# theblackcat102/edgedict

Hardware: NVIDIA H100
Metric: audio-sec/sec E6D2 B=32 T=1000 U=128 V=1024 training step (higher is better)
Workload: dtype bf16

## Files before the change

edgedict_b200/csrc/common.cuh:

```cuda
#pragma once
#include <cuda_runtime.h>
#include <cuda_bf16.h>
#include <stdint.h>
#include <stdio.h>
#include <math.h>

#define EB_OK 0
#define EB_ERR_INVALID 2
#define EB_ERR_CUDA 3

#define EB_API extern "C" __attribute__((visibility("default")))

#define EB_CHECK_LAUNCH()                                                             \
    do {                                                                              \
        cudaError_t e__ = cudaGetLastError();                                         \
        if (e__ != cudaSuccess) {                                                     \
            fprintf(stderr, "[edgedict_b200] %s:%d CUDA error: %s\n", __FILE__,       \
                    __LINE__, cudaGetErrorString(e__));                               \
            return EB_ERR_CUDA;                                                       \
        }                                                                             \
    } while (0)

#define EB_CUDA(call)                                                                 \
    do {                                                                              \
        cudaError_t e__ = (call);                                                     \
        if (e__ != cudaSuccess) {                                                     \
            fprintf(stderr, "[edgedict_b200] %s:%d CUDA error: %s\n", __FILE__,       \
                    __LINE__, cudaGetErrorString(e__));                               \
            return EB_ERR_CUDA;                                                       \
        }                                                                             \
    } while (0)

static inline int eb_num_sms() {
    static int n = 0;
    if (n == 0) {
        int dev = 0;
        cudaGetDevice(&dev);
        cudaDeviceGetAttribute(&n, cudaDevAttrMultiProcessorCount, dev);
        if (n <= 0) n = 132;
    }
    return n;
}

__device__ __forceinline__ float warp_max(float v) {
#pragma unroll
    for (int o = 16; o > 0; o >>= 1) v = fmaxf(v, __shfl_xor_sync(0xffffffffu, v, o));
    return v;
}
__device__ __forceinline__ double warp_max(double v) {
#pragma unroll
    for (int o = 16; o > 0; o >>= 1) v = fmax(v, __shfl_xor_sync(0xffffffffu, v, o));
    return v;
}
template <typename T>
__device__ __forceinline__ T warp_sum(T v) {
#pragma unroll
    for (int o = 16; o > 0; o >>= 1) v += __shfl_xor_sync(0xffffffffu, v, o);
    return v;
}

template <typename T>
__device__ __forceinline__ T block_sum(T v, T* sh ) {
    const int lane = threadIdx.x & 31, w = threadIdx.x >> 5;
    v = warp_sum(v);
    __syncthreads();
    if (lane == 0) sh[w] = v;
    __syncthreads();
    const int nw = (blockDim.x + 31) >> 5;
    T r = (threadIdx.x < nw) ? sh[threadIdx.x] : T(0);
    if (w == 0) {
        r = warp_sum(r);
        if (lane == 0) sh[32] = r;
    }
    __syncthreads();
    return sh[32];
}

__device__ __forceinline__ void spin_wait_ge(const unsigned* ctr, unsigned target) {
    unsigned v;
    long long t0 = 0;
    unsigned spins = 0;
    while (true) {
        asm volatile("ld.acquire.gpu.global.u32 %0, [%1];" : "=r"(v) : "l"(ctr) : "memory");
        if (v >= target) break;
        if ((++spins & 0xFFFF) == 0) {
            const long long now = clock64();
            if (t0 == 0) t0 = now;
            else if (now - t0 > 8000000000LL) {
                printf("[edgedict_b200] grid barrier timeout: block %d saw %u, wants %u\n", blockIdx.x, v, target);
                __trap();
            }
        }
    }
}

__device__ __forceinline__ float fast_ex2(float x) {
    float y;
    asm("ex2.approx.ftz.f32 %0, %1;" : "=f"(y) : "f"(x));
    return y;
}
__device__ __forceinline__ float fast_exp(float x) { return fast_ex2(x * 1.4426950408889634f); }
__device__ __forceinline__ float sigmoidf_(float x) { return 1.0f / (1.0f + expf(-x)); }

__device__ __forceinline__ float4 ld_stream_f4(const float* p) {
    float4 r;
    asm volatile("ld.global.nc.L1::no_allocate.v4.f32 {%0,%1,%2,%3}, [%4];"
                 : "=f"(r.x), "=f"(r.y), "=f"(r.z), "=f"(r.w) : "l"(p));
    return r;
}
__device__ __forceinline__ void st_stream_f4(float* p, float4 v) {
    asm volatile("st.global.L1::no_allocate.v4.f32 [%0], {%1,%2,%3,%4};"
                 :: "l"(p), "f"(v.x), "f"(v.y), "f"(v.z), "f"(v.w) : "memory");
}
```

edgedict_b200/csrc/gemm_tc.cu:

```cuda
#include <cuda.h>
#include <stdlib.h>
#include "common.cuh"
#include "sm90.cuh"
#include "../../include/edgedict_b200.h"

namespace {

constexpr int BM = 128, BK = 64, UMMA_K = 16;
constexpr int A_BYTES = BM * BK * 2;
constexpr int NTHREADS = 2 * 128 + 32;
template <int BN_, bool LOW_ = false> struct Cfg {
    static constexpr int STAGES = LOW_ ? 3 : (BN_ == 256 ? 4 : 6);
    static constexpr int B_BYTES = BN_ * BK * 2;
    static constexpr int STAGE_BYTES = A_BYTES + B_BYTES;
    static constexpr int SMEM_BYTES = 1024 + STAGES * STAGE_BYTES + 256;
};

struct Sched {
    long num_m; int num_n; int ksplit; long out_tiles; bool n_inner;
    unsigned wid, nw;
    __device__ __forceinline__ bool get(long j, long& m_blk, int& n_blk, int& ks) const {
        if (n_inner) {
            const long grp = (long)wid + (j / num_n) * nw;
            if (grp >= num_m) return false;
            m_blk = grp; n_blk = (int)(j % num_n); ks = 0;
            return true;
        }
        const long wi = (long)wid + j * nw;
        if (wi >= out_tiles * ksplit) return false;
        const long tile = wi % out_tiles;
        ks = (int)(wi / out_tiles);
        m_blk = tile / num_n; n_blk = (int)(tile % num_n);
        return true;
    }
};

struct LseArgs {
    const int* labels; const int* xlen; const int* ylen;
    float* denom; float* lpb; float* lpl;
    int maxT, maxU, blank;
    const __nv_bfloat16* aux;
};

__device__ __forceinline__ void st_bf16x2(__nv_bfloat16* p, float a, float b) {
    *reinterpret_cast<__nv_bfloat162*>(p) = __floats2bfloat162_rn(a, b);
}

template <bool A_MN, bool B_MN, int BN_, bool LSE = false, bool LOW_ = false>
__global__ void __launch_bounds__(NTHREADS, LOW_ ? 2 : 1)
gemm_tc_kernel(const __grid_constant__ CUtensorMap tma_a, const __grid_constant__ CUtensorMap tma_b,
               void* __restrict__ Cout, int c_bf16, const float* __restrict__ bias, int accumulate,
               long M, int N, long K, int ksplit, LseArgs lse = LseArgs(), float* __restrict__ part = nullptr) {
    using C_ = Cfg<BN_, LOW_>;
    constexpr int BN = BN_, STAGES = C_::STAGES, STAGE_BYTES = C_::STAGE_BYTES, NACC = BN / 2;
    extern __shared__ uint8_t smem_raw[];
    uint8_t* smem = reinterpret_cast<uint8_t*>((reinterpret_cast<uintptr_t>(smem_raw) + 1023) & ~uintptr_t(1023));
    uint8_t* tiles = smem;
    uint64_t* bars = reinterpret_cast<uint64_t*>(smem + STAGES * STAGE_BYTES);
    const uint32_t full0 = smem_u32(bars), empty0 = smem_u32(bars + STAGES);

    const int warp = threadIdx.x >> 5, lane = threadIdx.x & 31;
    const long num_m = (M + BM - 1) / BM;
    const int num_n = (N + BN - 1) / BN;
    Sched sch;
    sch.num_m = num_m; sch.num_n = num_n; sch.ksplit = ksplit; sch.out_tiles = num_m * num_n;
    sch.wid = blockIdx.x; sch.nw = gridDim.x;
    sch.n_inner = LSE || ((ksplit == 1) && (num_m >= 2L * sch.nw));
    const int nkb_total = (int)((K + BK - 1) / BK);
    const int kb_per = (nkb_total + ksplit - 1) / ksplit;

    if (threadIdx.x == 0) {
        for (int s = 0; s < STAGES; ++s) { mbar_init(full0 + 8 * s, 1); mbar_init(empty0 + 8 * s, 8); }
        asm volatile("fence.mbarrier_init.release.cluster;" ::: "memory");
        asm volatile("prefetch.tensormap [%0];" :: "l"(&tma_a) : "memory");
        asm volatile("prefetch.tensormap [%0];" :: "l"(&tma_b) : "memory");
    }
    __syncthreads();

    if (warp == 8) {
        if (lane == 0) {
            int stage = 0; uint32_t phase = 0;
            long mb; int nb, ksx;
            constexpr uint32_t TX = A_BYTES + C_::B_BYTES;
            for (long jj = 0; sch.get(jj, mb, nb, ksx); ++jj) {
                const int kb0 = ksx * kb_per, kb1 = min(nkb_total, kb0 + kb_per);
                const int m0 = (int)mb * BM, n0 = nb * BN;
                for (int kb = kb0; kb < kb1; ++kb) {
                    mbar_wait(empty0 + 8 * stage, phase ^ 1);
                    const uint32_t sa = smem_u32(tiles + stage * STAGE_BYTES), sb = sa + A_BYTES;
                    const uint32_t fb = full0 + 8 * stage;
                    mbar_expect_tx(fb, TX);
                    if (!A_MN) tma_load_2d(sa, &tma_a, kb * BK, m0, fb);
                    else { tma_load_2d(sa, &tma_a, m0, kb * BK, fb); tma_load_2d(sa + 8192, &tma_a, m0 + 64, kb * BK, fb); }
                    if (!B_MN) tma_load_2d(sb, &tma_b, kb * BK, n0, fb);
                    else {
#pragma unroll
                        for (int bx = 0; bx < BN / 64; ++bx) tma_load_2d(sb + bx * 8192, &tma_b, n0 + bx * 64, kb * BK, fb);
                    }
                    if (++stage == STAGES) { stage = 0; phase ^= 1; }
                }
            }
        }
        return;
    }

    const int wg = warp >> 2;
    const int r_in = 64 * wg + 16 * (warp & 3) + (lane >> 2);
    const int cq = 2 * (lane & 3);
    float* Cf = reinterpret_cast<float*>(Cout);
    __nv_bfloat16* const Ch = reinterpret_cast<__nv_bfloat16*>(Cout);
    const bool vec2 = (N % 2) == 0;
    float acc[NACC];
    int stage = 0; uint32_t phase = 0;
    long mb; int nb, ks;
    float rm[2] = {-INFINITY, -INFINITY}, rs[2] = {0.f, 0.f}, xb[2] = {0.f, 0.f}, xl[2] = {0.f, 0.f};
    int lab[2] = {-1, -1};
    bool cell_ok[2] = {false, false};
    for (long jj = 0; sch.get(jj, mb, nb, ks); ++jj) {
        const int kb0 = ks * kb_per, kb1 = min(nkb_total, kb0 + kb_per);
        const long m0 = mb * BM;
        const int n0 = nb * BN;
#pragma unroll
        for (int i = 0; i < NACC; ++i) acc[i] = 0.f;
        int prev = -1;
        for (int kb = kb0; kb < kb1; ++kb) {
            mbar_wait(full0 + 8 * stage, phase);
            const uint32_t sa = smem_u32(tiles + stage * STAGE_BYTES) + (uint32_t)wg * 8192u, sb = smem_u32(tiles + stage * STAGE_BYTES) + A_BYTES;
            wgmma_fence();
#pragma unroll
            for (int k = 0; k < BK / UMMA_K; ++k) {
                const uint64_t ad = A_MN ? make_desc(sa + k * 2048, 8192, 1024) : make_desc(sa + k * 32, 16, 1024);
                const uint64_t bd = B_MN ? make_desc(sb + k * 2048, 8192, 1024) : make_desc(sb + k * 32, 16, 1024);
                if constexpr (BN == 256) wgmma_m64n256k16<A_MN ? 1 : 0, B_MN ? 1 : 0>(acc, ad, bd, 1);
                else wgmma_m64n128k16<A_MN ? 1 : 0, B_MN ? 1 : 0>(acc, ad, bd, 1);
            }
            wgmma_commit();
            wgmma_wait<1>();
            if (prev >= 0 && lane == 0) mbar_arrive(empty0 + 8 * prev);
            prev = stage;
            if (++stage == STAGES) { stage = 0; phase ^= 1; }
        }
        wgmma_wait<0>();
        wgmma_fence_regs(acc);
        if (prev >= 0 && lane == 0) mbar_arrive(empty0 + 8 * prev);

        if constexpr (LSE) {
            constexpr float LOG2E = 1.4426950408889634f;
            if (nb == 0) {
#pragma unroll
                for (int h = 0; h < 2; ++h) {
                    rm[h] = -INFINITY; rs[h] = 0.f; xb[h] = 0.f; xl[h] = 0.f; lab[h] = -1; cell_ok[h] = false;
                    const long cell = m0 + r_in + 8 * h;
                    if (cell < M) {
                        const int u = (int)(cell % lse.maxU);
                        const long bt = cell / lse.maxU;
                        const int t = (int)(bt % lse.maxT), b = (int)(bt / lse.maxT);
                        const int Tn = lse.xlen[b], Un = lse.ylen[b] + 1;
                        cell_ok[h] = t < Tn && u < Un;
                        if (cell_ok[h] && u < Un - 1) lab[h] = lse.labels[b * (lse.maxU - 1) + u];
                    }
                }
            }
#pragma unroll
            for (int h = 0; h < 2; ++h) {
                float cm = -INFINITY;
#pragma unroll
                for (int i = 0; i < BN / 8; ++i) {
                    const int col = n0 + 8 * i + cq;
                    float v0 = acc[4 * i + 2 * h], v1 = acc[4 * i + 2 * h + 1];
                    v0 = col < N ? v0 + (bias ? __ldg(bias + col) : 0.f) : -INFINITY;
                    v1 = col + 1 < N ? v1 + (bias ? __ldg(bias + col + 1) : 0.f) : -INFINITY;
                    acc[4 * i + 2 * h] = v0; acc[4 * i + 2 * h + 1] = v1;
                    cm = fmaxf(cm, fmaxf(v0, v1));
                    if (col == lse.blank) xb[h] = v0;
                    if (col + 1 == lse.blank) xb[h] = v1;
                    if (col == lab[h]) xl[h] = v0;
                    if (col + 1 == lab[h]) xl[h] = v1;
                }
                const float nm = fmaxf(rm[h], cm);
                if (nm != -INFINITY) {
                    const float nml = nm * LOG2E;
                    float a0 = 0.f, a1 = 0.f;
#pragma unroll
                    for (int i = 0; i < BN / 8; ++i) {
                        a0 += fast_ex2(fmaf(acc[4 * i + 2 * h], LOG2E, -nml));
                        a1 += fast_ex2(fmaf(acc[4 * i + 2 * h + 1], LOG2E, -nml));
                    }
                    rs[h] = rs[h] * fast_ex2((rm[h] - nm) * LOG2E) + (a0 + a1);
                    rm[h] = nm;
                }
                const long row = m0 + r_in + 8 * h;
                if (row < M) {
#pragma unroll
                    for (int i = 0; i < BN / 8; ++i) {
                        const int col = n0 + 8 * i + cq;
                        __nv_bfloat16* cp = Ch + row * N + col;
                        if (vec2 && col + 1 < N) st_bf16x2(cp, acc[4 * i + 2 * h], acc[4 * i + 2 * h + 1]);
                        else {
                            if (col < N) cp[0] = __float2bfloat16(acc[4 * i + 2 * h]);
                            if (col + 1 < N) cp[1] = __float2bfloat16(acc[4 * i + 2 * h + 1]);
                        }
                    }
                }
            }
            if (nb == num_n - 1) {
#pragma unroll
                for (int h = 0; h < 2; ++h) {
#pragma unroll
                    for (int o = 1; o <= 2; o <<= 1) {
                        const float m2 = __shfl_xor_sync(0xffffffffu, rm[h], o), s2 = __shfl_xor_sync(0xffffffffu, rs[h], o);
                        xb[h] += __shfl_xor_sync(0xffffffffu, xb[h], o);
                        xl[h] += __shfl_xor_sync(0xffffffffu, xl[h], o);
                        const float m = fmaxf(rm[h], m2);
                        rs[h] = (rm[h] == -INFINITY ? 0.f : rs[h] * fast_ex2((rm[h] - m) * LOG2E)) +
                                (m2 == -INFINITY ? 0.f : s2 * fast_ex2((m2 - m) * LOG2E));
                        rm[h] = m;
                    }
                    if ((lane & 3) == 0 && cell_ok[h]) {
                        const long cell = m0 + r_in + 8 * h;
                        const float d = -(rm[h] + logf(rs[h]));
                        lse.denom[cell] = d;
                        lse.lpb[cell] = d + xb[h];
                        lse.lpl[cell] = d + xl[h];
                    }
                }
            }
        } else {
            const bool add_bias = bias && ks == 0;
            if (ksplit > 1) Cf = part + (long)ks * M * N;
            const int acc_c = ksplit > 1 ? 0 : accumulate;
#pragma unroll
            for (int h = 0; h < 2; ++h) {
                const long row = m0 + r_in + 8 * h;
                if (row >= M) continue;
                constexpr bool PRE = BN == 128 && !LOW_;
                __nv_bfloat162 hx[PRE ? BN / 8 : 1];
                if constexpr (PRE) {
                    if (c_bf16 && lse.aux) {
#pragma unroll
                        for (int i = 0; i < BN / 8; ++i) {
                            const int col = n0 + 8 * i + cq;
                            const long off = row * N + col;
                            hx[i] = __floats2bfloat162_rn(0.f, 0.f);
                            if (col + 1 < N && vec2) hx[i] = __ldg(reinterpret_cast<const __nv_bfloat162*>(lse.aux + off));
                            else if (col < N) {
                                hx[i].x = lse.aux[off];
                                if (col + 1 < N) hx[i].y = lse.aux[off + 1];
                            }
                        }
                    }
                }
#pragma unroll
                for (int i = 0; i < BN / 8; ++i) {
                    const int col = n0 + 8 * i + cq;
                    if (col >= N) break;
                    const bool two = col + 1 < N, pair = two && vec2;
                    float v0 = acc[4 * i + 2 * h], v1 = acc[4 * i + 2 * h + 1];
                    if (add_bias) { v0 += __ldg(bias + col); if (two) v1 += __ldg(bias + col + 1); }
                    const long off = row * N + col;
                    if (c_bf16) {
                        __nv_bfloat16* cp = Ch + off;
                        if (lse.aux) {
                            float h0, h1 = 0.f;
                            if constexpr (PRE) {
                                const float2 hh = __bfloat1622float2(hx[i]);
                                h0 = hh.x;
                                if (two) h1 = hh.y;
                            } else if (pair) {
                                const float2 hh = __bfloat1622float2(__ldg(reinterpret_cast<const __nv_bfloat162*>(lse.aux + off)));
                                h0 = hh.x; h1 = hh.y;
                            } else {
                                h0 = __bfloat162float(lse.aux[off]);
                                if (two) h1 = __bfloat162float(lse.aux[off + 1]);
                            }
                            v0 *= 1.f - h0 * h0; v1 *= 1.f - h1 * h1;
                        }
                        if (pair) {
                            if (accumulate) {
                                const float2 o = __bfloat1622float2(*reinterpret_cast<const __nv_bfloat162*>(cp));
                                v0 += o.x; v1 += o.y;
                            }
                            st_bf16x2(cp, v0, v1);
                        } else {
                            if (accumulate) { v0 += __bfloat162float(cp[0]); if (two) v1 += __bfloat162float(cp[1]); }
                            cp[0] = __float2bfloat16(v0);
                            if (two) cp[1] = __float2bfloat16(v1);
                        }
                    } else {
                        float* cp = Cf + off;
                        if (pair) {
                            if (acc_c) { const float2 o = *reinterpret_cast<const float2*>(cp); v0 += o.x; v1 += o.y; }
                            *reinterpret_cast<float2*>(cp) = make_float2(v0, v1);
                        } else {
                            if (acc_c) { v0 += cp[0]; if (two) v1 += cp[1]; }
                            cp[0] = v0;
                            if (two) cp[1] = v1;
                        }
                    }
                }
            }
        }
    }
}

__global__ void splitk_reduce_kernel(const float* __restrict__ part, int ksplit, long mn, float* __restrict__ C, int accumulate) {
    for (long i = (long)blockIdx.x * blockDim.x + threadIdx.x; i < mn; i += (long)gridDim.x * blockDim.x) {
        float v = accumulate ? C[i] : 0.f;
        for (int s = 0; s < ksplit; ++s) v += part[(long)s * mn + i];
        C[i] = v;
    }
}

int choose_ksplit(long out_tiles, long nkb, long workers, double r) {
    int ksplit = 1;
    long cap = nkb / 16;
    if (cap > 64) cap = 64;
    double best = -1.0;
    for (long ks = 1; ks <= cap; ++ks) {
        const long items = out_tiles * ks;
        const long waves = (items + workers - 1) / workers;
        const double score = (double)items / (double)(waves * workers) / (1.0 + r * (double)ks / (double)nkb);
        if (score > best) { best = score; ksplit = (int)ks; }
    }
    return ksplit;
}

template <bool A_MN, bool B_MN, int BN_, bool LSE, bool LOW_>
int launch_kernel(const CUtensorMap& ta, const CUtensorMap& tb, void* C, int c_bf16, const float* bias, int accumulate,
                  long M, int N, long K, int ksplit, long work, const LseArgs& ea, cudaStream_t st, float* part = nullptr) {
    using C_ = Cfg<BN_, LOW_>;
    auto kern = gemm_tc_kernel<A_MN, B_MN, BN_, LSE, LOW_>;
    static bool attr_done = false;
    if (!attr_done) {
        EB_CUDA(cudaFuncSetAttribute(kern, cudaFuncAttributeMaxDynamicSharedMemorySize, C_::SMEM_BYTES));
        attr_done = true;
    }
    const int grid = (int)(work < eb_num_sms() ? work : eb_num_sms());
    kern<<<grid, NTHREADS, C_::SMEM_BYTES, st>>>(ta, tb, C, c_bf16, bias, accumulate, M, N, K, ksplit, ea, part);
    EB_CHECK_LAUNCH();
    if (ksplit > 1) {
        const long mn = M * (long)N;
        const long blocks = (mn + 255) / 256, cap = 4L * eb_num_sms();
        splitk_reduce_kernel<<<(int)(blocks < cap ? blocks : cap), 256, 0, st>>>(part, ksplit, mn, (float*)C, accumulate);
        EB_CHECK_LAUNCH();
    }
    return EB_OK;
}

template <bool A_MN, bool B_MN, int BN_>
int launch(const CUtensorMap& ta, const CUtensorMap& tb, void* C, int c_bf16, const float* bias, int accumulate,
           long M, int N, long K, int ksplit, float* part, cudaStream_t st, const void* aux = nullptr) {
    LseArgs ea = LseArgs();
    ea.aux = reinterpret_cast<const __nv_bfloat16*>(aux);
    const long out_tiles = ((M + BM - 1) / BM) * ((N + BN_ - 1) / BN_);
    return launch_kernel<A_MN, B_MN, BN_, false, false>(ta, tb, C, c_bf16, bias, accumulate, M, N, K, ksplit,
                                                        out_tiles * ksplit, ea, st, part);
}

void plan(int a_mn_major, int c_bf16, int accumulate, long M, int N, long K, int flags, bool& wide, int& ksplit) {
    const bool low = (flags & EB_GEMM_CORESIDENT) != 0;
    static int force_bn = -1;
    if (force_bn < 0) { const char* e = getenv("EDGEDICT_GEMM_BN"); force_bn = e ? atoi(e) : 0; }
    const long wide_tiles = ((M + BM - 1) / BM) * (N / 256);
    wide = (N % 256 == 0) && (wide_tiles >= eb_num_sms() || (!c_bf16 && (K + BK - 1) / BK >= 64 && wide_tiles >= 8));
    if (!wide && N % 256 == 128 && N >= 512 && (M + BM - 1) / BM >= 4L * eb_num_sms() && accumulate == 0) wide = true;
    if (force_bn == 128) wide = false;
    if (force_bn == 256 && N % 128 == 0) wide = true;
    if (low) wide = false;
    (void)a_mn_major;
    const int BN = wide ? 256 : 128;
    const long out_tiles = ((M + BM - 1) / BM) * ((N + BN - 1) / BN);
    const long nkb = (K + BK - 1) / BK;
    ksplit = 1;
    if (!low && !c_bf16 && nkb >= 64 && out_tiles < eb_num_sms())
        ksplit = choose_ksplit(out_tiles, nkb, eb_num_sms(), BN == 256 ? 32.0 : 16.0);
}

int launch_low(const CUtensorMap& ta, const CUtensorMap& tb, void* C, int c_bf16, const float* bias, int accumulate,
               long M, int N, long K, cudaStream_t st) {
    const long tiles = ((M + BM - 1) / BM) * ((N + 127) / 128);
    return launch_kernel<false, false, 128, false, true>(ta, tb, C, c_bf16, bias, accumulate, M, N, K, 1, tiles, LseArgs(), st);
}

int launch_lse(const CUtensorMap& ta, const CUtensorMap& tb, void* C, const float* bias, long M, int N, long K,
               const LseArgs& lse, cudaStream_t st) {
    return launch_kernel<false, false, 128, true, false>(ta, tb, C, 1, bias, 0, M, N, K, 1, (M + BM - 1) / BM, lse, st);
}

}

EB_API int eb_joint_logits_lse(const void* hidden16, const void* w2_16, const float* b2, void* logits16,
                               const int* labels, const int* xlen, const int* ylen, float* denom, float* lpb,
                               float* lpl, int B, int maxT, int maxU, int V, int J, int blank, void* stream) {
    if (!hidden16 || !w2_16 || !logits16 || !xlen || !ylen || !denom || !lpb || !lpl || (!labels && maxU > 1) ||
        B <= 0 || maxT <= 0 || maxU <= 0 || V <= 0 || J <= 0 || J % 8 || blank < 0 || blank >= V)
        return EB_ERR_INVALID;
    if ((reinterpret_cast<uintptr_t>(hidden16) & 15) || (reinterpret_cast<uintptr_t>(w2_16) & 15) ||
        (b2 && (reinterpret_cast<uintptr_t>(b2) & 15)))
        return EB_ERR_INVALID;
    const long M = (long)B * maxT * maxU;
    CUtensorMap ta, tb;
    if (!make_map(&ta, hidden16, (uint64_t)J, (uint64_t)M, 128) || !make_map(&tb, w2_16, (uint64_t)J, (uint64_t)V, 128)) {
        fprintf(stderr, "[edgedict_b200] cuTensorMapEncodeTiled failed\n");
        return EB_ERR_CUDA;
    }
    LseArgs lse;
    lse.labels = labels; lse.xlen = xlen; lse.ylen = ylen; lse.denom = denom; lse.lpb = lpb; lse.lpl = lpl;
    lse.maxT = maxT; lse.maxU = maxU; lse.blank = blank; lse.aux = nullptr;
    cudaStream_t st = reinterpret_cast<cudaStream_t>(stream);
    return launch_lse(ta, tb, logits16, b2, M, V, J, lse, st);
}

EB_API int eb_gemm_bf16(const void* A, int a_mn_major, const void* B, int b_mn_major, void* C, int c_bf16,
                        const float* bias, int accumulate, long M, int N, long K, void* stream) {
    return eb_gemm_bf16_ex(A, a_mn_major, B, b_mn_major, C, c_bf16, bias, accumulate, M, N, K, 0, nullptr, 0, stream);
}

static int gemm_dispatch(const void* A, int a_mn_major, const void* B, int b_mn_major, void* C, int c_bf16,
                         const float* bias, int accumulate, long M, int N, long K, int flags, const void* aux,
                         float* partials, long partial_floats, void* stream);

EB_API long eb_gemm_bf16_partials(int a_mn_major, int c_bf16, int accumulate, long M, int N, long K, int flags) {
    if (M <= 0 || N <= 0 || K <= 0) return 0;
    bool wide;
    int ksplit;
    plan(a_mn_major, c_bf16, accumulate, M, N, K, flags, wide, ksplit);
    return ksplit > 1 ? (long)ksplit * M * N : 0;
}

EB_API int eb_gemm_bf16_ex(const void* A, int a_mn_major, const void* B, int b_mn_major, void* C, int c_bf16,
                           const float* bias, int accumulate, long M, int N, long K, int flags, float* partials,
                           long partial_floats, void* stream) {
    return gemm_dispatch(A, a_mn_major, B, b_mn_major, C, c_bf16, bias, accumulate, M, N, K, flags, nullptr, partials,
                         partial_floats, stream);
}

EB_API int eb_gemm_bf16_dtanh(const void* A, int a_mn_major, const void* B, int b_mn_major, void* C16,
                              const void* hid16, long M, int N, long K, void* stream) {
    if (!hid16 || (reinterpret_cast<uintptr_t>(hid16) & 7) || (reinterpret_cast<uintptr_t>(C16) & 7) || N % 4) return EB_ERR_INVALID;
    return gemm_dispatch(A, a_mn_major, B, b_mn_major, C16, 1, nullptr, 0, M, N, K, 0, hid16, nullptr, 0, stream);
}

static int gemm_dispatch(const void* A, int a_mn_major, const void* B, int b_mn_major, void* C, int c_bf16,
                         const float* bias, int accumulate, long M, int N, long K, int flags, const void* aux,
                         float* partials, long partial_floats, void* stream) {
    if (!A || !B || !C || M <= 0 || N <= 0 || K <= 0) return EB_ERR_INVALID;
    const bool low = (flags & EB_GEMM_CORESIDENT) != 0;
    if (low && (a_mn_major || b_mn_major)) return EB_ERR_INVALID;
    if ((reinterpret_cast<uintptr_t>(A) & 15) || (reinterpret_cast<uintptr_t>(B) & 15)) return EB_ERR_INVALID;
    if ((a_mn_major ? M : K) % 8 || (b_mn_major ? (long)N : K) % 8) return EB_ERR_INVALID;
    bool wide;
    int ksplit;
    plan(a_mn_major, c_bf16, accumulate, M, N, K, flags, wide, ksplit);
    if (aux) wide = false;
    if (ksplit > 1) {
        const long fit = (partials && (reinterpret_cast<uintptr_t>(partials) & 7) == 0) ? partial_floats / (M * (long)N) : 0;
        if (fit < ksplit) ksplit = fit > 1 ? (int)fit : 1;
    }
    CUtensorMap ta, tb;
    bool ok = a_mn_major ? make_map(&ta, A, (uint64_t)M, (uint64_t)K, 64) : make_map(&ta, A, (uint64_t)K, (uint64_t)M, 128);
    ok = ok && (b_mn_major ? make_map(&tb, B, (uint64_t)N, (uint64_t)K, 64)
                           : make_map(&tb, B, (uint64_t)K, (uint64_t)N, wide ? 256 : 128));
    if (!ok) {
        fprintf(stderr, "[edgedict_b200] cuTensorMapEncodeTiled failed\n");
        return EB_ERR_CUDA;
    }
    cudaStream_t st = reinterpret_cast<cudaStream_t>(stream);
    if (low) return launch_low(ta, tb, C, c_bf16, bias, accumulate, M, N, K, st);
#define EB_GO(AM, BMN)                                                                                          \
    return wide ? launch<AM, BMN, 256>(ta, tb, C, c_bf16, bias, accumulate, M, N, K, ksplit, partials, st, aux) \
                : launch<AM, BMN, 128>(ta, tb, C, c_bf16, bias, accumulate, M, N, K, ksplit, partials, st, aux)
    if (a_mn_major) {
        if (b_mn_major) { EB_GO(true, true); }
        EB_GO(true, false);
    }
    if (b_mn_major) { EB_GO(false, true); }
    EB_GO(false, false);
#undef EB_GO
}
```

edgedict_b200/csrc/sm90.cuh:

```cuda
#pragma once
#include <cuda.h>
#include "common.cuh"

namespace {

__device__ __forceinline__ uint32_t smem_u32(const void* p) { return (uint32_t)__cvta_generic_to_shared(p); }

__device__ __forceinline__ void mbar_init(uint32_t bar, uint32_t count) {
    asm volatile("mbarrier.init.shared::cta.b64 [%0], %1;" :: "r"(bar), "r"(count) : "memory");
}
__device__ __forceinline__ void mbar_expect_tx(uint32_t bar, uint32_t bytes) {
    asm volatile("mbarrier.arrive.expect_tx.shared::cta.b64 _, [%0], %1;" :: "r"(bar), "r"(bytes) : "memory");
}
__device__ __forceinline__ void mbar_arrive(uint32_t bar) {
    asm volatile("mbarrier.arrive.shared::cta.b64 _, [%0];" :: "r"(bar) : "memory");
}
__device__ __forceinline__ void mbar_wait(uint32_t bar, uint32_t parity) {
    uint32_t ok = 0;
    unsigned long long spins = 0;
    do {
        asm volatile("{\n .reg .pred p;\n mbarrier.try_wait.parity.shared::cta.b64 p, [%1], %2;\n"
                     " selp.u32 %0, 1, 0, p;\n}\n" : "=r"(ok) : "r"(bar), "r"(parity) : "memory");
        if (!ok && ++spins > (1ull << 26)) {
            printf("[edgedict_b200] mbarrier wait timeout (block %d warp %d)\n", blockIdx.x,
                   threadIdx.x >> 5);
            __trap();
        }
    } while (!ok);
}
__device__ __forceinline__ void tma_load_2d(uint32_t dst, const CUtensorMap* map, int c0, int c1, uint32_t bar) {
    asm volatile("cp.async.bulk.tensor.2d.shared::cluster.global.mbarrier::complete_tx::bytes [%0], [%1, {%3, %4}], [%2];"
                 :: "r"(dst), "l"(map), "r"(bar), "r"(c0), "r"(c1) : "memory");
}

__device__ __forceinline__ void wgmma_fence() { asm volatile("wgmma.fence.sync.aligned;" ::: "memory"); }
__device__ __forceinline__ void wgmma_commit() { asm volatile("wgmma.commit_group.sync.aligned;" ::: "memory"); }
template <int N>
__device__ __forceinline__ void wgmma_wait() { asm volatile("wgmma.wait_group.sync.aligned %0;" :: "n"(N) : "memory"); }
template <int R>
__device__ __forceinline__ void wgmma_fence_regs(float (&d)[R]) {
#pragma unroll
    for (int i = 0; i < R; ++i) asm volatile("" : "+f"(d[i]) :: "memory");
}
template <int TA, int TB>
__device__ __forceinline__ void wgmma_m64n32k16(float (&d)[16], uint64_t da, uint64_t db, int scale_d) {
    asm volatile("{\n .reg .pred p;\n setp.ne.b32 p, %18, 0;\n"
                 " wgmma.mma_async.sync.aligned.m64n32k16.f32.bf16.bf16 {"
                 "%0,%1,%2,%3,%4,%5,%6,%7,%8,%9,%10,%11,%12,%13,%14,%15"
                 "}, %16, %17, p, 1, 1, %19, %20;\n}\n"
                 : "+f"(d[0]), "+f"(d[1]), "+f"(d[2]), "+f"(d[3]), "+f"(d[4]), "+f"(d[5]), "+f"(d[6]), "+f"(d[7]),
                   "+f"(d[8]), "+f"(d[9]), "+f"(d[10]), "+f"(d[11]), "+f"(d[12]), "+f"(d[13]), "+f"(d[14]), "+f"(d[15])
                 : "l"(da), "l"(db), "r"(scale_d), "n"(TA), "n"(TB));
}
template <int TA, int TB>
__device__ __forceinline__ void wgmma_m64n128k16(float (&d)[64], uint64_t da, uint64_t db, int scale_d) {
    asm volatile("{\n .reg .pred p;\n setp.ne.b32 p, %66, 0;\n"
                 " wgmma.mma_async.sync.aligned.m64n128k16.f32.bf16.bf16 {"
                 "%0,%1,%2,%3,%4,%5,%6,%7,%8,%9,%10,%11,%12,%13,%14,%15,"
                 "%16,%17,%18,%19,%20,%21,%22,%23,%24,%25,%26,%27,%28,%29,%30,%31,"
                 "%32,%33,%34,%35,%36,%37,%38,%39,%40,%41,%42,%43,%44,%45,%46,%47,"
                 "%48,%49,%50,%51,%52,%53,%54,%55,%56,%57,%58,%59,%60,%61,%62,%63"
                 "}, %64, %65, p, 1, 1, %67, %68;\n}\n"
                 : "+f"(d[0]), "+f"(d[1]), "+f"(d[2]), "+f"(d[3]), "+f"(d[4]), "+f"(d[5]), "+f"(d[6]), "+f"(d[7]),
                   "+f"(d[8]), "+f"(d[9]), "+f"(d[10]), "+f"(d[11]), "+f"(d[12]), "+f"(d[13]), "+f"(d[14]), "+f"(d[15]),
                   "+f"(d[16]), "+f"(d[17]), "+f"(d[18]), "+f"(d[19]), "+f"(d[20]), "+f"(d[21]), "+f"(d[22]), "+f"(d[23]),
                   "+f"(d[24]), "+f"(d[25]), "+f"(d[26]), "+f"(d[27]), "+f"(d[28]), "+f"(d[29]), "+f"(d[30]), "+f"(d[31]),
                   "+f"(d[32]), "+f"(d[33]), "+f"(d[34]), "+f"(d[35]), "+f"(d[36]), "+f"(d[37]), "+f"(d[38]), "+f"(d[39]),
                   "+f"(d[40]), "+f"(d[41]), "+f"(d[42]), "+f"(d[43]), "+f"(d[44]), "+f"(d[45]), "+f"(d[46]), "+f"(d[47]),
                   "+f"(d[48]), "+f"(d[49]), "+f"(d[50]), "+f"(d[51]), "+f"(d[52]), "+f"(d[53]), "+f"(d[54]), "+f"(d[55]),
                   "+f"(d[56]), "+f"(d[57]), "+f"(d[58]), "+f"(d[59]), "+f"(d[60]), "+f"(d[61]), "+f"(d[62]), "+f"(d[63])
                 : "l"(da), "l"(db), "r"(scale_d), "n"(TA), "n"(TB));
}
template <int TA, int TB>
__device__ __forceinline__ void wgmma_m64n256k16(float (&d)[128], uint64_t da, uint64_t db, int scale_d) {
    asm volatile("{\n .reg .pred p;\n setp.ne.b32 p, %130, 0;\n"
                 " wgmma.mma_async.sync.aligned.m64n256k16.f32.bf16.bf16 {"
                 "%0,%1,%2,%3,%4,%5,%6,%7,%8,%9,%10,%11,%12,%13,%14,%15,"
                 "%16,%17,%18,%19,%20,%21,%22,%23,%24,%25,%26,%27,%28,%29,%30,%31,"
                 "%32,%33,%34,%35,%36,%37,%38,%39,%40,%41,%42,%43,%44,%45,%46,%47,"
                 "%48,%49,%50,%51,%52,%53,%54,%55,%56,%57,%58,%59,%60,%61,%62,%63,"
                 "%64,%65,%66,%67,%68,%69,%70,%71,%72,%73,%74,%75,%76,%77,%78,%79,"
                 "%80,%81,%82,%83,%84,%85,%86,%87,%88,%89,%90,%91,%92,%93,%94,%95,"
                 "%96,%97,%98,%99,%100,%101,%102,%103,%104,%105,%106,%107,%108,%109,%110,%111,"
                 "%112,%113,%114,%115,%116,%117,%118,%119,%120,%121,%122,%123,%124,%125,%126,%127"
                 "}, %128, %129, p, 1, 1, %131, %132;\n}\n"
                 : "+f"(d[0]), "+f"(d[1]), "+f"(d[2]), "+f"(d[3]), "+f"(d[4]), "+f"(d[5]), "+f"(d[6]), "+f"(d[7]),
                   "+f"(d[8]), "+f"(d[9]), "+f"(d[10]), "+f"(d[11]), "+f"(d[12]), "+f"(d[13]), "+f"(d[14]), "+f"(d[15]),
                   "+f"(d[16]), "+f"(d[17]), "+f"(d[18]), "+f"(d[19]), "+f"(d[20]), "+f"(d[21]), "+f"(d[22]), "+f"(d[23]),
                   "+f"(d[24]), "+f"(d[25]), "+f"(d[26]), "+f"(d[27]), "+f"(d[28]), "+f"(d[29]), "+f"(d[30]), "+f"(d[31]),
                   "+f"(d[32]), "+f"(d[33]), "+f"(d[34]), "+f"(d[35]), "+f"(d[36]), "+f"(d[37]), "+f"(d[38]), "+f"(d[39]),
                   "+f"(d[40]), "+f"(d[41]), "+f"(d[42]), "+f"(d[43]), "+f"(d[44]), "+f"(d[45]), "+f"(d[46]), "+f"(d[47]),
                   "+f"(d[48]), "+f"(d[49]), "+f"(d[50]), "+f"(d[51]), "+f"(d[52]), "+f"(d[53]), "+f"(d[54]), "+f"(d[55]),
                   "+f"(d[56]), "+f"(d[57]), "+f"(d[58]), "+f"(d[59]), "+f"(d[60]), "+f"(d[61]), "+f"(d[62]), "+f"(d[63]),
                   "+f"(d[64]), "+f"(d[65]), "+f"(d[66]), "+f"(d[67]), "+f"(d[68]), "+f"(d[69]), "+f"(d[70]), "+f"(d[71]),
                   "+f"(d[72]), "+f"(d[73]), "+f"(d[74]), "+f"(d[75]), "+f"(d[76]), "+f"(d[77]), "+f"(d[78]), "+f"(d[79]),
                   "+f"(d[80]), "+f"(d[81]), "+f"(d[82]), "+f"(d[83]), "+f"(d[84]), "+f"(d[85]), "+f"(d[86]), "+f"(d[87]),
                   "+f"(d[88]), "+f"(d[89]), "+f"(d[90]), "+f"(d[91]), "+f"(d[92]), "+f"(d[93]), "+f"(d[94]), "+f"(d[95]),
                   "+f"(d[96]), "+f"(d[97]), "+f"(d[98]), "+f"(d[99]), "+f"(d[100]), "+f"(d[101]), "+f"(d[102]), "+f"(d[103]),
                   "+f"(d[104]), "+f"(d[105]), "+f"(d[106]), "+f"(d[107]), "+f"(d[108]), "+f"(d[109]), "+f"(d[110]), "+f"(d[111]),
                   "+f"(d[112]), "+f"(d[113]), "+f"(d[114]), "+f"(d[115]), "+f"(d[116]), "+f"(d[117]), "+f"(d[118]), "+f"(d[119]),
                   "+f"(d[120]), "+f"(d[121]), "+f"(d[122]), "+f"(d[123]), "+f"(d[124]), "+f"(d[125]), "+f"(d[126]), "+f"(d[127])
                 : "l"(da), "l"(db), "r"(scale_d), "n"(TA), "n"(TB));
}


__device__ __forceinline__ uint64_t make_desc(uint32_t saddr, uint32_t lbo_bytes, uint32_t sbo_bytes) {
    uint64_t d = 0;
    d |= (uint64_t)((saddr & 0x3FFFF) >> 4);
    d |= (uint64_t)((lbo_bytes >> 4) & 0x3FFF) << 16;
    d |= (uint64_t)((sbo_bytes >> 4) & 0x3FFF) << 32;
    d |= (uint64_t)1 << 62;
    return d;
}


__device__ __forceinline__ uint32_t cluster_ctarank() {
    uint32_t r;
    asm volatile("mov.u32 %0, %%cluster_ctarank;" : "=r"(r));
    return r;
}
__device__ __forceinline__ uint32_t map_to_rank(uint32_t saddr, uint32_t rank) {
    uint32_t r;
    asm volatile("mapa.shared::cluster.u32 %0, %1, %2;" : "=r"(r) : "r"(saddr), "r"(rank));
    return r;
}
__device__ __forceinline__ void st_cluster_f4(uint32_t caddr, float a, float b, float c, float d) {
    asm volatile("st.shared::cluster.v4.f32 [%0], {%1,%2,%3,%4};" :: "r"(caddr), "f"(a), "f"(b), "f"(c), "f"(d) : "memory");
}
__device__ __forceinline__ void mbar_arrive_cluster(uint32_t caddr) {
    asm volatile("mbarrier.arrive.release.cluster.shared::cluster.b64 _, [%0];" :: "r"(caddr) : "memory");
}
__device__ __forceinline__ void mbar_wait_cluster(uint32_t bar, uint32_t parity) {
    uint32_t ok = 0;
    unsigned long long spins = 0;
    do {
        asm volatile("{\n .reg .pred p;\n mbarrier.try_wait.parity.acquire.cluster.shared::cta.b64 p, [%1], %2;\n"
                     " selp.u32 %0, 1, 0, p;\n}\n" : "=r"(ok) : "r"(bar), "r"(parity) : "memory");
        if (!ok && ++spins > (1ull << 26)) {
            printf("[edgedict_b200] cluster mbarrier wait timeout (block %d warp %d)\n", blockIdx.x, threadIdx.x >> 5);
            __trap();
        }
    } while (!ok);
}
__device__ __forceinline__ void cluster_sync_all() {
    asm volatile("barrier.cluster.arrive.release.aligned;\nbarrier.cluster.wait.acquire.aligned;" ::: "memory");
}
__device__ __forceinline__ void fence_proxy_async() { asm volatile("fence.proxy.async;" ::: "memory"); }

__device__ __forceinline__ void bulk_s2c(uint32_t dst_cluster, uint32_t src_cta, uint32_t bytes, uint32_t mbar_cluster) {
    asm volatile("cp.async.bulk.shared::cluster.shared::cta.mbarrier::complete_tx::bytes [%0], [%1], %2, [%3];"
                 :: "r"(dst_cluster), "r"(src_cta), "r"(bytes), "r"(mbar_cluster) : "memory");
}
__device__ __forceinline__ void fence_proxy_async_smem() { asm volatile("fence.proxy.async.shared::cta;" ::: "memory"); }

typedef CUresult (*EncodeTiledFn)(CUtensorMap*, CUtensorMapDataType, cuuint32_t, void*, const cuuint64_t*,
                                  const cuuint64_t*, const cuuint32_t*, const cuuint32_t*,
                                  CUtensorMapInterleave, CUtensorMapSwizzle, CUtensorMapL2promotion,
                                  CUtensorMapFloatOOBfill);

inline EncodeTiledFn get_encode() {
    static EncodeTiledFn fn = nullptr;
    if (!fn) {
        void* p = nullptr;
        cudaDriverEntryPointQueryResult q;
        if (cudaGetDriverEntryPoint("cuTensorMapEncodeTiled", &p, cudaEnableDefault, &q) != cudaSuccess ||
            q != cudaDriverEntryPointSuccess)
            return nullptr;
        fn = reinterpret_cast<EncodeTiledFn>(p);
    }
    return fn;
}

inline bool make_map(CUtensorMap* map, const void* ptr, uint64_t inner, uint64_t outer, uint32_t box_outer) {
    EncodeTiledFn enc = get_encode();
    if (!enc) return false;
    cuuint64_t dims[2] = {inner, outer};
    cuuint64_t strides[1] = {inner * 2};
    cuuint32_t box[2] = {64, box_outer};
    cuuint32_t estr[2] = {1, 1};
    CUresult r = enc(map, CU_TENSOR_MAP_DATA_TYPE_BFLOAT16, 2, const_cast<void*>(ptr), dims, strides, box, estr,
                     CU_TENSOR_MAP_INTERLEAVE_NONE, CU_TENSOR_MAP_SWIZZLE_128B, CU_TENSOR_MAP_L2_PROMOTION_L2_256B,
                     CU_TENSOR_MAP_FLOAT_OOB_FILL_NONE);
    return r == CUDA_SUCCESS;
}

}
```

edgedict_b200/functional.py:

```python
import torch

from . import ops

import os

f32, bf16 = torch.float32, torch.bfloat16
FUSE_JOINT_LSE = os.environ.get("EDGEDICT_FUSE_LSE", "1") != "0"


def _c(t):
    return t if t.is_contiguous() else t.contiguous()


class Linear(torch.autograd.Function):

    @staticmethod
    def forward(ctx, x, w, b, precision):
        shp = x.shape
        x2 = _c(x).view(-1, shp[-1])
        x16 = ops.cast_bf16(x2) if precision == "bf16" else None
        y = ops.mm_nt(x2, w, b, precision, x16=x16)
        ctx.save_for_backward(x2 if x16 is None else x16, w)
        ctx.precision, ctx.has_b, ctx.shp = precision, b is not None, shp
        return y.view(*shp[:-1], w.shape[0])

    @staticmethod
    def backward(ctx, dy):
        xs, w = ctx.saved_tensors
        p = ctx.precision
        dy2 = _c(dy).view(-1, dy.shape[-1])
        dy16 = ops.cast_bf16(dy2) if p == "bf16" else None
        dx = dw = db = None
        if ctx.needs_input_grad[0]:
            dx = ops.mm_nn(dy2, w, p, dy16=dy16).view(ctx.shp)
        if ctx.needs_input_grad[1]:
            dw = ops.mm_tn(dy2, xs, p, dy16=dy16, x16=xs if p == "bf16" else None)
        if ctx.has_b and ctx.needs_input_grad[2]:
            db = ops.colsum(dy2)
        return dx, dw, db, None


class LayerNormRes(torch.autograd.Function):

    @staticmethod
    def forward(ctx, x, res, gamma, beta, eps):
        x = _c(x)
        res = _c(res) if res is not None else None
        y, _, mean, rstd = ops.layernorm_fwd(x, res, gamma, beta, eps)
        ctx.save_for_backward(x, res, gamma, mean, rstd)
        return y

    @staticmethod
    def backward(ctx, dy):
        x, res, gamma, mean, rstd = ctx.saved_tensors
        dz, dgamma, dbeta = ops.layernorm_bwd(_c(dy), x, res, gamma, mean, rstd)
        return dz, (dz if res is not None else None), dgamma, dbeta, None


class TimeReduce(torch.autograd.Function):

    @staticmethod
    def forward(ctx, x):
        ctx.T = x.shape[1]
        y, _ = ops.time_reduce_fwd(_c(x))
        return y

    @staticmethod
    def backward(ctx, dy):
        return ops.time_reduce_bwd(_c(dy), ctx.T)


class Embedding(torch.autograd.Function):

    @staticmethod
    def forward(ctx, ids, w, prepend_bos, bos, pad):
        ids = _c(ids)
        if ids.dtype not in (torch.int32, torch.int64):
            ids = ids.long()
        ctx.save_for_backward(ids)
        ctx.meta = (w.shape[0], prepend_bos, bos, pad)
        return ops.embedding_fwd(ids, w, prepend_bos, bos)

    @staticmethod
    def backward(ctx, dout):
        (ids,) = ctx.saved_tensors
        V, prepend_bos, bos, pad = ctx.meta
        return None, ops.embedding_bwd(ids, _c(dout), V, prepend_bos, bos, pad), None, None, None


C4_BPTT_MIN_H = 1024


def _c4_bptt(H):
    return H >= C4_BPTT_MIN_H and ops.lstm_c4_bwd_chunks_supported(H)


class LSTMLayer(torch.autograd.Function):

    @staticmethod
    def forward(ctx, x, h0, c0, w_ih, w_hh, b_ih, b_hh, precision):
        B, T, I = x.shape
        H = w_hh.shape[1]
        x2 = _c(x).view(B * T, I)
        x16 = ops.cast_bf16(x2) if precision == "bf16" else None
        bias = b_ih + b_hh
        xg = ops.mm_nt(x2, w_ih, bias, precision, x16=x16).view(B, T, 4 * H)
        h0c = _c(h0) if h0 is not None else None
        c0c = _c(c0) if c0 is not None else None
        need = any(ctx.needs_input_grad)
        tc = precision == "bf16" and ops.lstm_tc_supported(B, H)
        c4 = precision == "bf16" and ops.lstm_c4_supported(B, H)
        if c4:
            y, y16, hT, cT, gates, cseq = ops.lstm_c4_fwd(xg, ops.cast_bf16(_c(w_hh)), h0c, c0c, need,
                                                          std_saves=None if ops.C4_BWD else True)
        elif tc:
            y, y16, hT, cT, gates, cseq = ops.lstm_tc_fwd(xg, ops.cast_bf16(_c(w_hh)), h0c, c0c, need)
        else:
            y, hT, cT, gates, cseq = ops.lstm_seq_fwd(xg, _c(w_hh), h0c, c0c, need)
            y16 = None
        if need:
            ctx.save_for_backward(x2 if x16 is None else x16, h0c, c0c, w_ih, w_hh, y16 if (tc or c4) else y, gates, cseq)
            ctx.precision, ctx.dims, ctx.tc, ctx.c4, ctx.c4_bwd = precision, (B, T, I, H), tc, c4, c4 and ops.C4_BWD
        return y, hT, cT

    @staticmethod
    def backward(ctx, dy, dhT, dcT):
        xs, h0, c0, w_ih, w_hh, y, gates, cseq = ctx.saved_tensors
        B, T, I, H = ctx.dims
        p = ctx.precision
        dy = _c(dy) if dy is not None else torch.zeros(B, T, H, dtype=f32, device=y.device)
        dhT = _c(dhT) if dhT is not None else None
        dcT = _c(dcT) if dcT is not None else None
        if getattr(ctx, "consumed", False):
            raise RuntimeError("LSTMLayer.backward ran twice on the same graph: the saved gates are overwritten in "
                               "place by the first pass (retain_graph is not supported by this node)")
        ctx.consumed = True
        if ctx.c4_bwd:
            dg16, dh0, dc0 = ops.lstm_c4_bwd(dy, gates, cseq, c0, ops.transpose_to_bf16(_c(w_hh)), dhT, dcT)
            dg2 = dg16.view(B * T, 4 * H)
        elif ctx.c4 and _c4_bptt(H):
            dg16, dh0, dc0 = ops.lstm_c4_bwd_chunks(dy, gates, cseq, ops.transpose_to_bf16(_c(w_hh)), [T], B,
                                                    torch.empty(B, T, 4 * H, dtype=bf16, device=dy.device), c0, dhT, dcT)
            dg2 = dg16.view(B * T, 4 * H)
        elif ctx.tc or ctx.c4:
            dg16, dh0, dc0 = ops.lstm_tc_bwd(dy, gates, cseq, c0, ops.transpose_to_bf16(_c(w_hh)), dhT, dcT)
            dg2 = dg16.view(B * T, 4 * H)
        else:
            dg, dh0, dc0 = ops.lstm_seq_bwd(dy, gates, cseq, c0, _c(w_hh), dhT, dcT)
            dg2 = dg.view(B * T, 4 * H)
            dg16 = ops.cast_bf16(dg2) if p == "bf16" else None
        dg16 = dg16.view(B * T, 4 * H) if dg16 is not None else None
        if ctx.c4:
            hp2 = y.view(B * T, H)
        else:
            hprev = torch.empty_like(y)
            hprev[:, 1:] = y[:, :-1]
            if h0 is not None:
                hprev[:, 0] = h0
            else:
                hprev[:, 0].zero_()
            hp2 = hprev.view(B * T, H)
        dx = ops.mm_nn(dg2, w_ih, p, dy16=dg16).view(B, T, I) if ctx.needs_input_grad[0] else None
        dw_ih = ops.mm_tn(dg2, xs, p, dy16=dg16, x16=xs if p == "bf16" else None)
        dw_hh = ops.mm_tn(dg2, hp2, p, dy16=dg16, x16=hp2 if hp2.dtype == bf16 else None)
        db = ops.colsum(dg2)
        return (dx, dh0 if ctx.needs_input_grad[1] else None, dc0 if ctx.needs_input_grad[2] else None,
                dw_ih, dw_hh, db, db.clone(), None)


class GRULayer(torch.autograd.Function):

    @staticmethod
    def forward(ctx, x, h0, w_ih, w_hh, b_ih, b_hh, precision):
        B, T, I = x.shape
        H = w_hh.shape[1]
        x2 = _c(x).view(B * T, I)
        x16 = ops.cast_bf16(x2) if precision == "bf16" else None
        bias = torch.cat([b_ih[:2 * H] + b_hh[:2 * H], b_ih[2 * H:]])
        xg = ops.mm_nt(x2, w_ih, bias, precision, x16=x16).view(B, T, 3 * H)
        h0c = _c(h0) if h0 is not None else None
        bhn = _c(b_hh[2 * H:])
        need = any(ctx.needs_input_grad)
        tc = precision == "bf16" and ops.gru_tc_supported(B, H)
        if tc:
            y, hT, save = ops.gru_tc_fwd(xg, ops.cast_bf16(_c(w_hh)), bhn, h0c, need)
        else:
            y, hT, save = ops.gru_seq_fwd(xg, _c(w_hh), bhn, h0c, need)
        if need:
            ctx.save_for_backward(x2 if x16 is None else x16, h0c, w_ih, w_hh, y, save)
            ctx.precision, ctx.dims, ctx.tc = precision, (B, T, I, H), tc
        return y, hT

    @staticmethod
    def backward(ctx, dy, dhT):
        xs, h0, w_ih, w_hh, y, save = ctx.saved_tensors
        B, T, I, H = ctx.dims
        p = ctx.precision
        if getattr(ctx, "consumed", False):
            raise RuntimeError("GRULayer.backward ran twice on the same graph (retain_graph is not supported by this "
                               "node)")
        ctx.consumed = True
        dy = _c(dy) if dy is not None else torch.zeros(B, T, H, dtype=f32, device=y.device)
        dhT = _c(dhT) if dhT is not None else None
        if ctx.tc:
            dgi, dgh, dh0 = ops.gru_tc_bwd(dy, save, y, h0, ops.transpose_to_bf16(_c(w_hh)), dhT)
        else:
            dgi, dgh, dh0 = ops.gru_seq_bwd(dy, save, y, h0, _c(w_hh), dhT)
        dgi2, dgh2 = dgi.view(B * T, 3 * H), dgh.view(B * T, 3 * H)
        dgi16 = (dgi2 if ctx.tc else ops.cast_bf16(dgi2)) if p == "bf16" else None
        dgh16 = (dgh2 if ctx.tc else ops.cast_bf16(dgh2)) if p == "bf16" else None
        hprev = torch.empty_like(y)
        hprev[:, 1:] = y[:, :-1]
        if h0 is not None:
            hprev[:, 0] = h0
        else:
            hprev[:, 0].zero_()
        hp2 = hprev.view(B * T, H)
        dx = ops.mm_nn(dgi2, w_ih, p, dy16=dgi16).view(B, T, I) if ctx.needs_input_grad[0] else None
        dw_ih = ops.mm_tn(dgi2, xs, p, dy16=dgi16, x16=xs if p == "bf16" else None)
        dw_hh = ops.mm_tn(dgh2, hp2, p, dy16=dgh16)
        return (dx, dh0 if ctx.needs_input_grad[1] else None, dw_ih, dw_hh, ops.colsum(dgi2), ops.colsum(dgh2), None)


WAVEFRONT_CHUNKS = int(os.environ.get("EDGEDICT_WAVEFRONT_CHUNKS", "6"))
_wave_streams = {}


def _side_streams(device):
    st = _wave_streams.get(device)
    if st is None:
        st = _wave_streams[device] = (torch.cuda.Stream(device), torch.cuda.Stream(device))
    return st


_aux_streams = {}


def _wave_aux_streams(device):
    st = _aux_streams.get(device)
    if st is None:
        st = _aux_streams[device] = tuple(torch.cuda.Stream(device) for _ in range(4))
    return st


def wavefront_plan(T, reductions, max_chunks=None):
    max_chunks = WAVEFRONT_CHUNKS if max_chunks is None else max_chunks
    if max_chunks < 2:
        return None
    gran = 1 << sum(1 for r in reductions if r)
    step = -(-T // (max_chunks * gran)) * gran
    if step < 16 * gran:
        step = 16 * gran
    lens = [min(step, T - t0) for t0 in range(0, T, step)]
    if len(lens) < 2:
        return None
    plan = [lens]
    for r in reductions:
        lens = [(n + 1) // 2 for n in lens] if r else lens
        plan.append(lens)
    return plan


class _Chunks:

    def __init__(self, B, lens):
        self.B, self.lens = B, lens
        self.off = [0]
        for n in lens:
            self.off.append(self.off[-1] + n)
        self.rows = B * self.off[-1]

    def new(self, D, dtype, device):
        return torch.empty(self.rows, D, dtype=dtype, device=device) if D else torch.empty(self.rows, dtype=dtype, device=device)

    def blk(self, buf, c):
        a, b = self.B * self.off[c], self.B * self.off[c + 1]
        v = buf[a:b]
        return v.view(self.B, self.lens[c], buf.shape[1]) if buf.dim() == 2 else v

    def scatter(self, x):
        out = self.new(x.shape[2], x.dtype, x.device)
        for c in range(len(self.lens)):
            self.blk(out, c).copy_(x[:, self.off[c]:self.off[c + 1]])
        return out

    def gather(self, buf):
        out = torch.empty(self.B, self.off[-1], buf.shape[1], dtype=buf.dtype, device=buf.device)
        for c in range(len(self.lens)):
            out[:, self.off[c]:self.off[c + 1]].copy_(self.blk(buf, c))
        return out


BPTT_ONE_LAUNCH = __import__("os").environ.get("EDGEDICT_BPTT_ONE_LAUNCH", "1") != "0"


class LSTMStack(torch.autograd.Function):

    collect = None

    @staticmethod
    def forward(ctx, x, cfg, *params):
        reductions, eps, plan = cfg
        L = len(reductions)
        B, T, I0 = x.shape
        dev = x.device
        H = params[1].shape[1]
        C = len(plan[0])
        need = any(ctx.needs_input_grad)
        c4 = ops.lstm_c4_supported(B, H)
        c4b = c4 and ops.C4_BWD
        ck = [_Chunks(B, lens) for lens in plan]
        P = [params[6 * l:6 * l + 6] for l in range(L)]
        wih16 = [ops.cast_bf16(_c(p[0])) for p in P]
        whh16 = [ops.cast_bf16(_c(p[1])) for p in P]
        bias = [p[2] + p[3] for p in P]
        x16 = [ck[0].scatter(ops.cast_bf16(_c(x)))] + [None] * L
        xs = [None] * (L + 1)
        y, y16, gates, cseq, mean, rstd = ([None] * L for _ in range(6))
        z = [None] * L
        for l in range(L):
            k, kn = ck[l], ck[l + 1]
            y[l] = k.new(H, f32, dev)
            y16[l] = k.new(H, bf16, dev) if (need or not c4) else None
            gates[l] = k.new(4 * H, f32, dev) if (need and not c4b) else None
            cseq[l] = k.new(H, f32, dev) if (need and not c4b) else None
            mean[l], rstd[l] = k.new(0, f32, dev), k.new(0, f32, dev)
            xs[l + 1] = kn.new(H, f32, dev)
            z[l] = k.new(H, f32, dev) if reductions[l] else xs[l + 1]
            x16[l + 1] = kn.new(H, bf16, dev) if l + 1 < L else None
        hT = torch.empty(L, C, B, H, dtype=f32, device=dev)
        cT = torch.empty(L, C, B, H, dtype=f32, device=dev)
        xgbuf = [[torch.empty(B * max(plan[l]), 4 * H, dtype=f32, device=dev) for _ in range(2)] for l in range(L)]
        c4saves = [[None] * C for _ in range(L)]

        main = torch.cuda.current_stream(dev)
        rec = _side_streams(dev)
        aux = _wave_aux_streams(dev)
        gem, nrm = aux[:2], aux[2:]
        ev = lambda: torch.cuda.Event()
        prep_done = [[ev() for _ in range(C)] for _ in range(L)]
        rec_done = [[ev() for _ in range(C)] for _ in range(L)]
        done = [[ev() for _ in range(C)] for _ in range(L)]
        for s_ in (*rec, *aux):
            s_.wait_stream(main)
        for d in range(L + C - 1):
            for l in range(max(0, d - C + 1), min(L, d + 1)):
                c = d - l
                k, kn = ck[l], ck[l + 1]
                Tc = k.lens[c]
                xg = xgbuf[l][c % 2][:B * Tc]
                with torch.cuda.stream(gem[l % 2]):
                    if l > 0:
                        gem[l % 2].wait_event(done[l - 1][c])
                    if c >= 2:
                        gem[l % 2].wait_event(rec_done[l][c - 2])
                    xin = k.blk(x16[l], c)
                    ops.gemm_bf16(xin.view(B * Tc, xin.shape[2]), 0, wih16[l], 0, B * Tc, 4 * H, xin.shape[2],
                                  bias=bias[l], out=xg, flags=ops.GEMM_CORESIDENT)
                    prep_done[l][c].record(gem[l % 2])
                with torch.cuda.stream(rec[l % 2]):
                    rec[l % 2].wait_event(prep_done[l][c])
                    if c4:
                        r = ops.lstm_c4_fwd(xg.view(B, Tc, 4 * H), whh16[l], hT[l, c - 1] if c else None,
                                            cT[l, c - 1] if c else None, need,
                                            out=(k.blk(y[l], c), k.blk(y16[l], c) if need else None, hT[l, c], cT[l, c]),
                                            std_saves=None if (c4b or not need) else (k.blk(gates[l], c), k.blk(cseq[l], c)))
                        if need and c4b:
                            c4saves[l][c] = (r[4], r[5])
                            r[4].record_stream(main)
                            r[5].record_stream(main)
                    else:
                        ops.lstm_tc_fwd(xg.view(B, Tc, 4 * H), whh16[l], hT[l, c - 1] if c else None,
                                        cT[l, c - 1] if c else None, need,
                                        out=(k.blk(y[l], c), k.blk(y16[l], c), hT[l, c], cT[l, c],
                                             k.blk(gates[l], c) if need else None, k.blk(cseq[l], c) if need else None))
                    rec_done[l][c].record(rec[l % 2])
                with torch.cuda.stream(nrm[l % 2]):
                    nrm[l % 2].wait_event(rec_done[l][c])
                    res = k.blk(xs[l], c) if l else None
                    nx16 = kn.blk(x16[l + 1], c) if x16[l + 1] is not None else None
                    if reductions[l]:
                        ops.layernorm_fwd(k.blk(y[l], c), res, P[l][4], P[l][5], eps[l],
                                          out=(k.blk(z[l], c), None, k.blk(mean[l], c), k.blk(rstd[l], c)))
                        ops.time_reduce_fwd(k.blk(z[l], c), out=(kn.blk(xs[l + 1], c), nx16))
                    else:
                        ops.layernorm_fwd(k.blk(y[l], c), res, P[l][4], P[l][5], eps[l],
                                          out=(kn.blk(xs[l + 1], c), nx16, k.blk(mean[l], c), k.blk(rstd[l], c)))
                    done[l][c].record(nrm[l % 2])
        for s_ in (*rec, *aux):
            main.wait_stream(s_)
        out = ck[L].gather(xs[L])
        if LSTMStack.collect is not None:
            LSTMStack.collect.extend(ck[l + 1].gather(xs[l + 1]) for l in range(L))
        hT_last, cT_last = hT[:, C - 1].contiguous(), cT[:, C - 1].contiguous()
        if need:
            if c4b:
                gates = [torch.empty(0, device=dev)] * L
                cseq = [torch.empty(0, device=dev)] * L
            flat_saves = [t for row in c4saves for pair in row for t in pair] if c4b else []
            ctx.save_for_backward(*params, hT, cT, *x16[:L], *xs[1:L], *y, *y16, *gates, *cseq, *mean, *rstd, *flat_saves)
            ctx.cfg, ctx.dims, ctx.c4, ctx.c4b = cfg, (B, T, I0, H, L, C), c4, c4b
        ctx.mark_non_differentiable(hT_last, cT_last)
        return out, hT_last, cT_last

    @staticmethod
    def backward(ctx, dout, _dh, _dc):
        reductions, eps, plan = ctx.cfg
        B, T, I0, H, L, C = ctx.dims
        sv = list(ctx.saved_tensors)
        params, sv = sv[:6 * L], sv[6 * L:]
        hT, cT = sv[0], sv[1]
        sv = sv[2:]
        x16, sv = sv[:L], sv[L:]
        xs, sv = [None] + sv[:L - 1], sv[L - 1:]
        y, y16, gates, cseq, mean, rstd = (sv[i * L:(i + 1) * L] for i in range(6))
        c4, c4b = ctx.c4, ctx.c4b
        flat_saves = sv[6 * L:]
        if getattr(ctx, "consumed", False):
            raise RuntimeError("LSTMStack.backward ran twice on the same graph (retain_graph is not supported)")
        ctx.consumed = True
        P = [params[6 * l:6 * l + 6] for l in range(L)]
        ck = [_Chunks(B, lens) for lens in plan]
        dev = dout.device
        main = torch.cuda.current_stream(dev)
        side = _side_streams(dev)[0]
        side.wait_stream(main)
        g = ck[L].scatter(_c(dout))
        grads = [None] * (6 * L)
        for l in range(L - 1, -1, -1):
            k, kn = ck[l], ck[l + 1]
            if reductions[l]:
                gz = k.new(H, f32, dev)
                for c in range(C):
                    ops.time_reduce_bwd(kn.blk(g, c), k.lens[c], out=k.blk(gz, c))
                g = gz
            dz, dgamma, dbeta = ops.layernorm_bwd(g, y[l], xs[l], P[l][4], mean[l], rstd[l])
            whhT16 = ops.transpose_to_bf16(_c(P[l][1]))
            dg16 = k.new(4 * H, bf16, dev)
            dh = dc = None
            if c4b:
                hprev = y16[l]
                for c in range(C - 1, -1, -1):
                    gs, cs = flat_saves[2 * (l * C + c)], flat_saves[2 * (l * C + c) + 1]
                    _, dh, dc = ops.lstm_c4_bwd(k.blk(dz, c), gs, cs, cT[l, c - 1] if c else None, whhT16, dh, dc,
                                                out=k.blk(dg16, c))
            else:
                hprev = y16[l] if c4 else k.new(H, bf16, dev)
                one_launch = c4 and BPTT_ONE_LAUNCH and C <= 8
                if one_launch and _c4_bptt(H):
                    ops.lstm_c4_bwd_chunks(dz, gates[l], cseq[l], whhT16, k.lens, B, dg16)
                elif one_launch:
                    ops.lstm_tc_bwd_chunks(dz, gates[l], cseq[l], whhT16, k.lens, B, dg16)
                for c in (() if one_launch else range(C - 1, -1, -1)):
                    _, dh, dc = ops.lstm_tc_bwd(k.blk(dz, c), k.blk(gates[l], c), k.blk(cseq[l], c),
                                                cT[l, c - 1] if c else None, whhT16, dh, dc, out=k.blk(dg16, c))
                    if c4:
                        continue
                    hp, yc = k.blk(hprev, c), k.blk(y16[l], c)
                    hp[:, 1:] = yc[:, :-1]
                    if c:
                        hp[:, 0] = k.blk(y16[l], c - 1)[:, -1]
                    else:
                        hp[:, 0].zero_()
            wih16 = ops.cast_bf16(_c(P[l][0]))
            M, I_l = dg16.shape[0], P[l][0].shape[1]
            if l > 0:
                g = ops.gemm_bf16(dg16, 0, wih16, 1, M, I_l, 4 * H, out=dz, accumulate=True, tag="gemm_bf16_nn")
            elif ctx.needs_input_grad[0]:
                g = ops.gemm_bf16(dg16, 0, wih16, 1, M, I_l, 4 * H, tag="gemm_bf16_nn")
            else:
                g = None
            ready = torch.cuda.Event()
            ready.record(main)
            with torch.cuda.stream(side):
                side.wait_event(ready)
                grads[6 * l + 0] = ops.mm_tn(dg16, x16[l], "bf16", dy16=dg16, x16=x16[l])
                grads[6 * l + 1] = ops.mm_tn(dg16, hprev, "bf16", dy16=dg16, x16=hprev)
                db = ops.colsum(dg16)
                grads[6 * l + 2], grads[6 * l + 3] = db, db.clone()
                for t_ in (dg16, hprev):
                    t_.record_stream(side)
                for t_ in grads[6 * l:6 * l + 4]:
                    t_.record_stream(main)
            grads[6 * l + 4], grads[6 * l + 5] = dgamma, dbeta
        main.wait_stream(side)
        dxin = ck[0].gather(g) if g is not None else None
        return (dxin, None, *grads)


def _joint_pre(h_enc, h_dec, w1, b1, precision):
    B, T, E = h_enc.shape
    U, Dd = h_dec.shape[1], h_dec.shape[2]
    J = w1.shape[0]
    he2, hd2 = _c(h_enc).view(B * T, E), _c(h_dec).view(B * U, Dd)
    ep = ops.mm_nt(he2, w1[:, :E], b1, precision).view(B, T, J)
    dp = ops.mm_nt(hd2, w1[:, E:], None, precision).view(B, U, J)
    return he2, hd2, ep, dp


JOINT_WGRAD_SIDE = __import__("os").environ.get("EDGEDICT_JOINT_WGRAD_SIDE", "1") != "0"


def _joint_bwd(ctx_p, dlog2, hid, he2, hd2, w1, w2, dims, db2=None):
    B, T, U, E, Dd, J, V = dims
    p = ctx_p
    dl16 = dlog2 if dlog2.dtype == bf16 else (ops.cast_bf16(dlog2) if p == "bf16" else None)
    hid2 = hid.view(B * T * U, J)

    def out_layer_grads(db2):
        if db2 is None:
            db2 = ops.colsum(dlog2)
        if p == "bf16" and V % 256 == 0:
            dw2 = ops.mm_tn(hid2, dl16, p, dy16=hid2, x16=dl16).t().contiguous()
        else:
            dw2 = ops.mm_tn(dlog2, hid2, p, dy16=dl16, x16=hid2 if p == "bf16" else None)
        return dw2, db2

    side = None
    if JOINT_WGRAD_SIDE and p == "bf16" and dlog2.is_cuda:
        main = torch.cuda.current_stream(dlog2.device)
        side = _side_streams(dlog2.device)[1]
        side.wait_stream(main)
        with torch.cuda.stream(side):
            dw2, db2 = out_layer_grads(db2)
        for t_ in (dlog2, dl16, hid2):
            if t_ is not None:
                t_.record_stream(side)
    else:
        dw2, db2 = out_layer_grads(db2)
    if p == "bf16" and J % 8 == 0 and hid.dtype == bf16:
        dpre = ops.gemm_bf16_dtanh(dl16, ops.cast_bf16(w2.contiguous()), True, hid2, B * T * U, J, V)
        dep, ddp = ops.joint_dpre_reduce(dpre.view(B, T, U, J))
    else:
        dhid = ops.mm_nn(dlog2, w2, p, dy16=dl16, out_bf16=(p == "bf16"))
        dep, ddp = ops.joint_hidden_bwd(dhid.view(B, T, U, J), hid)
    dep2, ddp2 = dep.view(B * T, J), ddp.view(B * U, J)
    w1e, w1d = w1[:, :E], w1[:, E:]
    dhe = ops.mm_nn(dep2, w1e, p).view(B, T, E)
    dhd = ops.mm_nn(ddp2, w1d, p).view(B, U, Dd)
    dw1 = torch.empty_like(w1)
    dw1[:, :E] = ops.mm_tn(dep2, he2, p)
    dw1[:, E:] = ops.mm_tn(ddp2, hd2, p)
    db1 = ops.colsum(dep2)
    if side is not None:
        main.wait_stream(side)
        dw2.record_stream(main)
        db2.record_stream(main)
    return dhe, dhd, dw1, db1, dw2, db2


class JointLogits(torch.autograd.Function):

    @staticmethod
    def forward(ctx, h_enc, h_dec, w1, b1, w2, b2, precision):
        B, T, E = h_enc.shape
        U, Dd = h_dec.shape[1], h_dec.shape[2]
        J, V = w1.shape[0], w2.shape[0]
        he2, hd2, ep, dp = _joint_pre(h_enc, h_dec, w1, b1, precision)
        hid = ops.joint_hidden_fwd(ep, dp, precision == "bf16")
        logits = ops.mm_nt(hid.view(B * T * U, J), w2, b2, precision, x16=hid.view(B * T * U, J) if precision == "bf16" else None)
        ctx.save_for_backward(hid, he2, hd2, w1, w2)
        ctx.precision, ctx.dims = precision, (B, T, U, E, Dd, J, V)
        return logits.view(B, T, U, V)

    @staticmethod
    def backward(ctx, dlogits):
        hid, he2, hd2, w1, w2 = ctx.saved_tensors
        B, T, U, E, Dd, J, V = ctx.dims
        dl2 = _c(dlogits).view(B * T * U, V)
        dhe, dhd, dw1, db1, dw2, db2 = _joint_bwd(ctx.precision, dl2, hid, he2, hd2, w1, w2, ctx.dims)
        return dhe, dhd, dw1, db1, dw2, db2, None


class RNNTLossFn(torch.autograd.Function):

    @staticmethod
    def forward(ctx, acts, labels, act_lens, label_lens, blank, reduction):
        acts = _c(acts)
        costs, ws = ops.rnnt_loss_fwd(acts, labels, act_lens, label_lens, blank, need_beta=True)
        B = acts.shape[0]
        ctx.save_for_backward(acts, labels, act_lens, label_lens, ws)
        ctx.blank, ctx.reduction, ctx.B = blank, reduction, B
        if reduction in ("sum", "mean"):
            costs = costs.sum().unsqueeze(-1)
            if reduction == "mean":
                costs = costs / B
        return costs

    @staticmethod
    def backward(ctx, go):
        acts, labels, act_lens, label_lens, ws = ctx.saved_tensors
        scale = 1.0 / ctx.B if ctx.reduction == "mean" else 1.0
        g = _c(go.to(acts.dtype)).view(-1)
        grads = ops.rnnt_loss_bwd(acts, labels, act_lens, label_lens, ctx.blank, ws, g, scale)
        return grads, None, None, None, None, None


class JointLoss(torch.autograd.Function):

    @staticmethod
    def forward(ctx, h_enc, h_dec, w1, b1, w2, b2, labels, act_lens, label_lens, blank, precision):
        B, T, E = h_enc.shape
        U, Dd = h_dec.shape[1], h_dec.shape[2]
        J, V = w1.shape[0], w2.shape[0]
        he2, hd2, ep, dp = _joint_pre(h_enc, h_dec, w1, b1, precision)
        hid = ops.joint_hidden_fwd(ep, dp, precision == "bf16")
        hid2 = hid.view(B * T * U, J)
        fused = precision == "bf16" and FUSE_JOINT_LSE and J % 8 == 0 and U <= 1024
        if fused:
            b2a = b2 if (b2.is_contiguous() and b2.data_ptr() % 16 == 0) else b2.clone()
            logits, ws = ops.joint_logits_lse(hid2, ops.cast_bf16(w2.contiguous()), b2a, labels, act_lens,
                                              label_lens, B, T, U, blank)
            costs = ops.rnnt_lattice(act_lens, label_lens, B, T, U, ws)
        else:
            logits = ops.mm_nt(hid2, w2, b2, precision, x16=hid2 if precision == "bf16" else None).view(B, T, U, V)
            costs, ws = ops.rnnt_loss_fwd(logits, labels, act_lens, label_lens, blank, need_beta=True)
        ctx.save_for_backward(hid, he2, hd2, w1, w2, logits, labels, act_lens, label_lens, ws)
        ctx.precision, ctx.dims, ctx.blank = precision, (B, T, U, E, Dd, J, V), blank
        ctx.mark_non_differentiable(costs)
        loss = costs.sum().unsqueeze(-1) / B
        ctx.costs = costs
        return loss, costs

    @staticmethod
    def backward(ctx, go, _gc):
        hid, he2, hd2, w1, w2, logits, labels, act_lens, label_lens, ws = ctx.saved_tensors
        if getattr(ctx, "consumed", False):
            raise RuntimeError("JointLoss.backward ran twice on the same graph: the gradient is written in place over "
                               "the saved logits (retain_graph is not supported by this node)")
        ctx.consumed = True
        B, T, U, E, Dd, J, V = ctx.dims
        p = ctx.precision
        g = _c(go.to(f32)).view(-1)
        if logits.dtype == bf16:
            dl = ops.rnnt_loss_bwd_bf16(logits, labels, act_lens, label_lens, ctx.blank, ws, g, 1.0 / B)
        elif p == "bf16":
            dl = ops.rnnt_loss_bwd(logits, labels, act_lens, label_lens, ctx.blank, ws, g, 1.0 / B, out_bf16=True)
        else:
            dl = ops.rnnt_loss_bwd(logits, labels, act_lens, label_lens, ctx.blank, ws, g, 1.0 / B, out=logits)
        dhe, dhd, dw1, db1, dw2, db2 = _joint_bwd(p, dl.view(B * T * U, V), hid, he2, hd2, w1, w2, ctx.dims)
        return dhe, dhd, dw1, db1, dw2, db2, None, None, None, None, None
```

edgedict_b200/ops.py:

```python
import torch

from ._lib import lib
from ._lib import check as _check


def _s():
    return torch.cuda.current_stream().cuda_stream


def _p(t):
    if t is None:
        return None
    if not t.is_cuda:
        raise RuntimeError("edgedict_b200 ops need CUDA tensors (got a %s tensor); there is no CPU path" % t.device)
    return t.data_ptr()


def _need(t, dtype=None, name="tensor"):
    if not t.is_cuda:
        raise RuntimeError("edgedict_b200 ops need CUDA tensors (%s is on %s); there is no CPU path" % (name, t.device))
    if dtype is not None and t.dtype != dtype:
        raise TypeError("%s must be %s, got %s" % (name, dtype, t.dtype))
    if not t.is_contiguous():
        raise ValueError("%s must be contiguous" % name)
    return t


f32, bf16 = torch.float32, torch.bfloat16


class _Prof:

    def __init__(self):
        self.enabled = False
        self.events = []
        self.launches = 0

    def reset(self):
        self.events, self.launches = [], 0

    def summary(self, base=None):
        out, spans = {}, {}
        for name, a, b, nbytes, flops in self.events:
            d = out.setdefault(name, dict(ms=0.0, ms_sum=0.0, calls=0, bytes=0.0, flops=0.0))
            d["ms_sum"] += a.elapsed_time(b)
            d["calls"] += 1
            d["bytes"] += nbytes
            d["flops"] += flops
            if base is not None:
                spans.setdefault(name, []).append((base.elapsed_time(a), base.elapsed_time(b)))
        for name, d in out.items():
            if base is None:
                d["ms"] = d["ms_sum"]
                continue
            tot, cur_s, cur_e = 0.0, None, None
            for s0, e0 in sorted(spans[name]):
                if cur_e is None or s0 > cur_e:
                    if cur_e is not None:
                        tot += cur_e - cur_s
                    cur_s, cur_e = s0, e0
                else:
                    cur_e = max(cur_e, e0)
            if cur_e is not None:
                tot += cur_e - cur_s
            d["ms"] = tot
        return out


PROF = _Prof()


def check(rc, what):
    PROF.launches += 1
    _check(rc, what)


class _timed:
    def __init__(self, name, kernels=1, nbytes=0.0, flops=0.0):
        self.name, self.k, self.nbytes, self.flops = name, kernels, nbytes, flops

    def __enter__(self):
        if PROF.enabled:
            self.a = torch.cuda.Event(enable_timing=True)
            self.a.record()
        return self

    def __exit__(self, *exc):
        PROF.launches += self.k - 1
        if PROF.enabled:
            b = torch.cuda.Event(enable_timing=True)
            b.record()
            PROF.events.append((self.name, self.a, b, self.nbytes, self.flops))
        return False


def cast_bf16(x, out=None):
    _need(x, f32, "x")
    y = out if out is not None else torch.empty(x.shape, dtype=bf16, device=x.device)
    n = x.numel()
    if n:
        check(lib().eb_cast_bf16(_p(x), _p(y), n, _s()), "eb_cast_bf16")
    return y


def gemm_f32(A, sam, sak, B, sbk, sbn, M, N, K, bias=None, out=None, beta=0.0, alpha=1.0):
    if out is None:
        out = torch.empty(M, N, dtype=f32, device=A.device)
    with _timed("gemm_f32", 1, 0.0, 2.0 * M * N * K):
        check(lib().eb_gemm_f32(_p(A), sam, sak, _p(B), sbk, sbn, _p(out), N, _p(bias), M, N, K, alpha, beta, _s()),
              "eb_gemm_f32")
    return out


GEMM_CORESIDENT = 1


def gemm_bf16(A, a_mn, B, b_mn, M, N, K, bias=None, out=None, out_bf16=False, accumulate=False, tag=None, flags=0):
    if out is None:
        out = torch.empty(M, N, dtype=bf16 if out_bf16 else f32, device=A.device)
    name = tag or ("gemm_bf16_%s%s" % ("t" if a_mn else "n", "n" if b_mn else "t"))
    with _timed(name, 1, 2.0 * (M * K + N * K) + out.element_size() * M * N, 2.0 * M * N * K):
        c16 = int(out.dtype == bf16)
        nws = int(lib().eb_gemm_bf16_partials(int(a_mn), c16, int(accumulate), M, N, K, int(flags)))
        ws = torch.empty(nws, dtype=f32, device=A.device) if nws else None
        check(lib().eb_gemm_bf16_ex(_p(A), int(a_mn), _p(B), int(b_mn), _p(out), c16, _p(bias), int(accumulate), M, N, K,
                                    int(flags), _p(ws), nws, _s()), "eb_gemm_bf16")
    return out


def mm_nt(x, w, bias=None, precision="fp32", x16=None, w16=None, out_bf16=False):
    M, K = x.shape
    N = w.shape[0]
    if precision == "bf16":
        x16 = x16 if x16 is not None else (x if x.dtype == bf16 else cast_bf16(x))
        w16 = w16 if w16 is not None else cast_bf16(w.contiguous())
        return gemm_bf16(x16, 0, w16, 0, M, N, K, bias=bias, out_bf16=out_bf16)
    _need(x, f32, "x")
    return gemm_f32(x, K, 1, w, w.stride(1), w.stride(0), M, N, K, bias=bias)


def mm_nn(dy, w, precision="fp32", dy16=None, w16=None, out_bf16=False):
    M, N = dy.shape
    K = w.shape[1]
    if precision == "bf16":
        dy16 = dy16 if dy16 is not None else (dy if dy.dtype == bf16 else cast_bf16(dy))
        w16 = w16 if w16 is not None else cast_bf16(w.contiguous())
        return gemm_bf16(dy16, 0, w16, 1, M, K, N, out_bf16=out_bf16)
    _need(dy, f32, "dy")
    return gemm_f32(dy, N, 1, w, w.stride(0), w.stride(1), M, K, N)


def mm_tn(dy, x, precision="fp32", dy16=None, x16=None, out=None, accumulate=False):
    M, N = dy.shape
    K = x.shape[1]
    if precision == "bf16":
        dy16 = dy16 if dy16 is not None else (dy if dy.dtype == bf16 else cast_bf16(dy))
        x16 = x16 if x16 is not None else (x if x.dtype == bf16 else cast_bf16(x))
        return gemm_bf16(dy16, 1, x16, 1, N, K, M, out=out, accumulate=accumulate)
    _need(dy, f32, "dy")
    _need(x, f32, "x")
    return gemm_f32(dy, 1, N, x, K, 1, N, K, M, out=out, beta=1.0 if accumulate else 0.0)


def colsum(x, out=None):
    rows, N = x.shape
    if out is None:
        out = torch.zeros(N, dtype=f32, device=x.device)
    check(lib().eb_colsum(_p(x), int(x.dtype == bf16), _p(out), rows, N, _s()), "eb_colsum")
    return out


def layernorm_fwd(x, res, gamma, beta, eps=1e-5, want_bf16=False, out=None):
    H = x.shape[-1]
    rows = x.numel() // H
    if out is not None:
        y, y16, mean, rstd = out
    else:
        y = torch.empty_like(x)
        y16 = torch.empty(x.shape, dtype=bf16, device=x.device) if want_bf16 else None
        mean = torch.empty(rows, dtype=f32, device=x.device)
        rstd = torch.empty(rows, dtype=f32, device=x.device)
    check(lib().eb_layernorm_fwd(_p(x), _p(res), _p(gamma), _p(beta), _p(y), _p(y16), _p(mean), _p(rstd),
                                 rows, H, eps, _s()), "eb_layernorm_fwd")
    return y, y16, mean, rstd


def layernorm_bwd(dy, x, res, gamma, mean, rstd):
    H = x.shape[-1]
    rows = x.numel() // H
    dz = torch.empty_like(x)
    dgamma = torch.zeros(H, dtype=f32, device=x.device)
    dbeta = torch.zeros(H, dtype=f32, device=x.device)
    check(lib().eb_layernorm_bwd(_p(dy), _p(x), _p(res), _p(gamma), _p(mean), _p(rstd), _p(dz), _p(dgamma),
                                 _p(dbeta), rows, H, _s()), "eb_layernorm_bwd")
    return dz, dgamma, dbeta


def time_reduce_fwd(x, want_bf16=False, out=None):
    B, T, H = x.shape
    if out is not None:
        y, y16 = out
    else:
        y = torch.empty(B, (T + 1) // 2, H, dtype=f32, device=x.device)
        y16 = torch.empty(y.shape, dtype=bf16, device=x.device) if want_bf16 else None
    check(lib().eb_time_reduce_fwd(_p(x), _p(y), _p(y16), B, T, H, _s()), "eb_time_reduce_fwd")
    return y, y16


def time_reduce_bwd(dy, T, out=None):
    B, _, H = dy.shape
    dx = out if out is not None else torch.empty(B, T, H, dtype=f32, device=dy.device)
    check(lib().eb_time_reduce_bwd(_p(dy), _p(dx), B, T, H, _s()), "eb_time_reduce_bwd")
    return dx


def embedding_fwd(ids, W, prepend_bos, bos):
    B, U = ids.shape
    E = W.shape[1]
    out = torch.empty(B, U + (1 if prepend_bos else 0), E, dtype=f32, device=W.device)
    if out.numel():
        check(lib().eb_embedding_fwd(_p(ids), int(ids.dtype == torch.int64), _p(W), _p(out), None, B, U, E,
                                     int(prepend_bos), bos, _s()), "eb_embedding_fwd")
    return out


def embedding_bwd(ids, dout, V, prepend_bos, bos, pad):
    B, U = ids.shape
    E = dout.shape[-1]
    dW = torch.zeros(V, E, dtype=f32, device=dout.device)
    if dout.numel():
        check(lib().eb_embedding_bwd(_p(ids), int(ids.dtype == torch.int64), _p(dout), _p(dW), B, U, E,
                                     int(prepend_bos), bos, pad, _s()), "eb_embedding_bwd")
    return dW


_scratch = {}


def _lstm_scratch(B, H, device):
    key = (B, H, device, _s())
    t = _scratch.get(key)
    if t is None:
        n = lib().eb_lstm_scratch_bytes(B, H)
        if n == 0:
            raise ValueError("LSTM hidden size %d not supported by the persistent kernel" % H)
        t = torch.zeros(n, dtype=torch.uint8, device=device)
        _scratch[key] = t
    return t


def lstm_seq_fwd(xg, whh, h0, c0, save):
    B, T, H4 = xg.shape
    H = H4 // 4
    dev = xg.device
    y = torch.empty(B, T, H, dtype=f32, device=dev)
    hT = torch.empty(B, H, dtype=f32, device=dev)
    cT = torch.empty(B, H, dtype=f32, device=dev)
    gates = torch.empty(B, T, H4, dtype=f32, device=dev) if save else None
    cseq = torch.empty(B, T, H, dtype=f32, device=dev) if save else None
    with _timed("lstm_seq_fwd", 1, 0.0, 2.0 * B * T * 4 * H * H):
        check(lib().eb_lstm_seq_fwd(_p(xg), _p(whh), _p(h0), _p(c0), _p(y), _p(hT), _p(cT), _p(gates), _p(cseq),
                                    _p(_lstm_scratch(B, H, dev)), B, T, H, _s()), "eb_lstm_seq_fwd")
    return y, hT, cT, gates, cseq


def lstm_seq_bwd(dy, gates, cseq, c0, whh, dhT, dcT):
    B, T, H = dy.shape
    dev = dy.device
    dh0 = torch.empty(B, H, dtype=f32, device=dev)
    dc0 = torch.empty(B, H, dtype=f32, device=dev)
    with _timed("lstm_seq_bwd", 1, 0.0, 2.0 * B * T * 4 * H * H):
        check(lib().eb_lstm_seq_bwd(_p(dy), _p(gates), _p(cseq), _p(c0), _p(whh), _p(dhT), _p(dcT), _p(gates),
                                    _p(dh0), _p(dc0), _p(_lstm_scratch(B, H, dev)), B, T, H, _s()), "eb_lstm_seq_bwd")
    return gates, dh0, dc0


def _gru_scratch(B, H, device):
    key = ("gru", B, H, device, _s())
    t = _scratch.get(key)
    if t is None:
        n = lib().eb_gru_scratch_bytes(B, H)
        if n == 0:
            raise ValueError("GRU hidden size %d not supported by the persistent kernel" % H)
        t = torch.zeros(n, dtype=torch.uint8, device=device)
        _scratch[key] = t
    return t


def gru_seq_fwd(xg, whh, bhn, h0, save):
    B, T, H3 = xg.shape
    H = H3 // 3
    dev = xg.device
    y = torch.empty(B, T, H, dtype=f32, device=dev)
    hT = torch.empty(B, H, dtype=f32, device=dev)
    sv = torch.empty(B, T, 4 * H, dtype=f32, device=dev) if save else None
    with _timed("gru_seq_fwd", 1, 0.0, 2.0 * B * T * 3 * H * H):
        check(lib().eb_gru_seq_fwd(_p(xg), _p(whh), _p(bhn), _p(h0), _p(y), _p(hT), _p(sv),
                                   _p(_gru_scratch(B, H, dev)), B, T, H, _s()), "eb_gru_seq_fwd")
    return y, hT, sv


def gru_seq_bwd(dy, save, y, h0, whh, dhT):
    B, T, H = dy.shape
    dev = dy.device
    dgi = torch.empty(B, T, 3 * H, dtype=f32, device=dev)
    dgh = torch.empty(B, T, 3 * H, dtype=f32, device=dev)
    dh0 = torch.empty(B, H, dtype=f32, device=dev)
    with _timed("gru_seq_bwd", 1, 0.0, 2.0 * B * T * 3 * H * H):
        check(lib().eb_gru_seq_bwd(_p(dy), _p(save), _p(y), _p(h0), _p(whh), _p(dhT), _p(dgi), _p(dgh), _p(dh0),
                                   _p(_gru_scratch(B, H, dev)), B, T, H, _s()), "eb_gru_seq_bwd")
    return dgi, dgh, dh0


def gru_tc_supported(B, H):
    return bool(lib().eb_gru_tc_supported(B, H))


def _gru_tc_scratch(B, H, device):
    key = ("gru_tc", H, device, _s())
    t = _scratch.get(key)
    if t is None:
        t = torch.zeros(lib().eb_gru_tc_scratch_bytes(B, H), dtype=torch.uint8, device=device)
        _scratch[key] = t
    return t


def gru_tc_fwd(xg, whh16, bhn, h0, save):
    B, T, H3 = xg.shape
    H = H3 // 3
    dev = xg.device
    y = torch.empty(B, T, H, dtype=f32, device=dev)
    hT = torch.empty(B, H, dtype=f32, device=dev)
    sv = torch.empty(B, T, 4 * H, dtype=f32, device=dev) if save else None
    with _timed("gru_tc_fwd", 1, 0.0, 2.0 * B * T * 3 * H * H):
        check(lib().eb_gru_tc_fwd(_p(xg), _p(whh16), _p(bhn), _p(h0), _p(y), _p(hT), _p(sv),
                                  _p(_gru_tc_scratch(B, H, dev)), B, T, H, _s()), "eb_gru_tc_fwd")
    return y, hT, sv


def gru_tc_bwd(dy, save, y, h0, whhT16, dhT):
    B, T, H = dy.shape
    dev = dy.device
    dgi = torch.empty(B, T, 3 * H, dtype=bf16, device=dev)
    dgh = torch.empty(B, T, 3 * H, dtype=bf16, device=dev)
    dh0 = torch.empty(B, H, dtype=f32, device=dev)
    with _timed("gru_tc_bwd", 1, 0.0, 2.0 * B * T * 3 * H * H):
        check(lib().eb_gru_tc_bwd(_p(dy), _p(save), _p(y), _p(h0), _p(whhT16), _p(dhT), _p(dgi), _p(dgh), _p(dh0),
                                  _p(_gru_tc_scratch(B, H, dev)), B, T, H, _s()), "eb_gru_tc_bwd")
    return dgi, dgh, dh0


def lstm_tc_supported(B, H):
    return bool(lib().eb_lstm_tc_supported(B, H))


def _lstm_tc_scratch(B, H, device):
    key = ("tc", H, device, _s())
    t = _scratch.get(key)
    if t is None:
        t = torch.zeros(lib().eb_lstm_tc_scratch_bytes(B, H), dtype=torch.uint8, device=device)
        _scratch[key] = t
    return t


def lstm_tc_fwd(xg, whh16, h0, c0, save, out=None):
    B, T, H4 = xg.shape
    H = H4 // 4
    dev = xg.device
    if out is not None:
        y, y16, hT, cT, gates, cseq = out
    else:
        y = torch.empty(B, T, H, dtype=f32, device=dev)
        y16 = torch.empty(B, T, H, dtype=bf16, device=dev)
        hT = torch.empty(B, H, dtype=f32, device=dev)
        cT = torch.empty(B, H, dtype=f32, device=dev)
        gates = torch.empty(B, T, H4, dtype=f32, device=dev) if save else None
        cseq = torch.empty(B, T, H, dtype=f32, device=dev) if save else None
    with _timed("lstm_tc_fwd", 1, 0.0, 2.0 * B * T * 4 * H * H):
        check(lib().eb_lstm_tc_fwd(_p(xg), _p(whh16), _p(h0), _p(c0), _p(y), _p(y16), _p(hT), _p(cT), _p(gates),
                                   _p(cseq), _p(_lstm_tc_scratch(B, H, dev)), B, T, H, _s()), "eb_lstm_tc_fwd")
    return y, y16, hT, cT, gates, cseq


def lstm_tc_bwd(dy, gates, cseq, c0, whhT16, dhT, dcT, out=None):
    B, T, H = dy.shape
    dev = dy.device
    dg16 = out if out is not None else torch.empty(B, T, 4 * H, dtype=bf16, device=dev)
    dh0 = torch.empty(B, H, dtype=f32, device=dev)
    dc0 = torch.empty(B, H, dtype=f32, device=dev)
    with _timed("lstm_tc_bwd", 1, 0.0, 2.0 * B * T * 4 * H * H):
        check(lib().eb_lstm_tc_bwd(_p(dy), _p(gates), _p(cseq), _p(c0), _p(whhT16), _p(dhT), _p(dcT), _p(dg16),
                                   _p(dh0), _p(dc0), _p(_lstm_tc_scratch(B, H, dev)), B, T, H, _s()), "eb_lstm_tc_bwd")
    return dg16, dh0, dc0


def lstm_tc_bwd_chunks(dy, gates, cseq, whhT16, lens, B, out):
    import ctypes
    H = dy.shape[1]
    dev = dy.device
    dh0 = torch.empty(B, H, dtype=f32, device=dev)
    dc0 = torch.empty(B, H, dtype=f32, device=dev)
    arr = (ctypes.c_int * len(lens))(*[int(n) for n in lens])
    with _timed("lstm_tc_bwd", 1, 0.0, 2.0 * B * sum(lens) * 4 * H * H):
        check(lib().eb_lstm_tc_bwd_chunks(_p(dy), _p(gates), _p(cseq), None, _p(whhT16), None, None, _p(out), _p(dh0),
                                          _p(dc0), _p(_lstm_tc_scratch(B, H, dev)), B, arr, len(lens), H, _s()),
              "eb_lstm_tc_bwd_chunks")
    return out, dh0, dc0


_c4_ok = {}


def lstm_c4_supported(B, H):
    v = _c4_ok.get(H)
    if v is None:
        v = _c4_ok[H] = bool(lib().eb_lstm_c4_supported(B, H))
    return v


def _lstm_c4_scratch(B, H, device):
    key = ("c4", H, device, _s())
    t = _scratch.get(key)
    if t is None:
        t = torch.zeros(lib().eb_lstm_c4_scratch_bytes(B, H), dtype=torch.uint8, device=device)
        _scratch[key] = t
    return t


def lstm_c4_save_buffers(B, T, H, device):
    return (torch.empty(lib().eb_lstm_c4_gsave_bytes(B, T, H), dtype=torch.uint8, device=device),
            torch.empty(lib().eb_lstm_c4_csave_bytes(B, T, H), dtype=torch.uint8, device=device))


C4_BWD = __import__("os").environ.get("EDGEDICT_LSTM_C4_BWD", "0") != "0"


def lstm_c4_fwd(xg, whh16, h0, c0, save, out=None, std_saves=None):
    B, T, H4 = xg.shape
    H = H4 // 4
    dev = xg.device
    if out is not None:
        y, hprev16, hT, cT = out
    else:
        y = torch.empty(B, T, H, dtype=f32, device=dev)
        hprev16 = torch.empty(B, T, H, dtype=bf16, device=dev) if save else None
        hT = torch.empty(B, H, dtype=f32, device=dev)
        cT = torch.empty(B, H, dtype=f32, device=dev)
    gsave = csave = gstd = cstd = None
    if save and std_saves is not None and std_saves is not False:
        gstd, cstd = std_saves if isinstance(std_saves, tuple) else (torch.empty(B, T, H4, dtype=f32, device=dev),
                                                                     torch.empty(B, T, H, dtype=f32, device=dev))
    elif save:
        gsave, csave = lstm_c4_save_buffers(B, T, H, dev)
    with _timed("lstm_tc_fwd", 1, 0.0, 2.0 * B * T * 4 * H * H):
        check(lib().eb_lstm_c4_fwd(_p(xg), _p(whh16), _p(h0), _p(c0), _p(y), _p(hprev16), _p(hT), _p(cT), _p(gsave),
                                   _p(csave), _p(gstd), _p(cstd), _p(_lstm_c4_scratch(B, H, dev)), B, T, H, _s()),
              "eb_lstm_c4_fwd")
    if gstd is not None:
        return y, hprev16, hT, cT, gstd, cstd
    return y, hprev16, hT, cT, gsave, csave


_c4_chunks_ok = {}


def lstm_c4_bwd_chunks_supported(H):
    v = _c4_chunks_ok.get(H)
    if v is None:
        v = _c4_chunks_ok[H] = lib().eb_lstm_c4_bwd_chunks_cluster(H) == 16
    return v


def lstm_c4_bwd_chunks(dy, gates, cseq, whhT16, lens, B, out, c0=None, dhT=None, dcT=None):
    import ctypes
    H = dy.shape[-1]
    dev = dy.device
    dh0 = torch.empty(B, H, dtype=f32, device=dev)
    dc0 = torch.empty(B, H, dtype=f32, device=dev)
    arr = (ctypes.c_int * len(lens))(*[int(n) for n in lens])
    with _timed("lstm_tc_bwd", 1, 0.0, 2.0 * B * sum(lens) * 4 * H * H):
        check(lib().eb_lstm_c4_bwd_chunks(_p(dy), _p(gates), _p(cseq), _p(c0), _p(whhT16), _p(dhT), _p(dcT), _p(out),
                                          _p(dh0), _p(dc0), _p(_lstm_c4_scratch(B, H, dev)), B, arr, len(lens), H, _s()),
              "eb_lstm_c4_bwd_chunks")
    return out, dh0, dc0


def lstm_c4_bwd(dy, gsave, csave, c0, whhT16, dhT, dcT, out=None):
    B, T, H = dy.shape
    dev = dy.device
    dg16 = out if out is not None else torch.empty(B, T, 4 * H, dtype=bf16, device=dev)
    dh0 = torch.empty(B, H, dtype=f32, device=dev)
    dc0 = torch.empty(B, H, dtype=f32, device=dev)
    with _timed("lstm_tc_bwd", 1, 0.0, 2.0 * B * T * 4 * H * H):
        check(lib().eb_lstm_c4_bwd(_p(dy), _p(gsave), _p(csave), _p(c0), _p(whhT16), _p(dhT), _p(dcT), _p(dg16),
                                   _p(dh0), _p(dc0), _p(_lstm_c4_scratch(B, H, dev)), B, T, H, _s()), "eb_lstm_c4_bwd")
    return dg16, dh0, dc0


def transpose_to_bf16(x):
    rows, cols = x.shape
    y = torch.empty(cols, rows, dtype=bf16, device=x.device)
    check(lib().eb_transpose_to_bf16(_p(x), int(x.dtype == bf16), _p(y), rows, cols, _s()), "eb_transpose_to_bf16")
    return y


def joint_hidden_fwd(ep, dp, want_bf16):
    B, T, J = ep.shape
    U = dp.shape[1]
    hid = torch.empty(B, T, U, J, dtype=bf16 if want_bf16 else f32, device=ep.device)
    check(lib().eb_joint_hidden_fwd(_p(ep), _p(dp), _p(hid), int(want_bf16), B, T, U, J, _s()), "eb_joint_hidden_fwd")
    return hid


def joint_hidden_bwd(dhid, hid):
    B, T, U, J = hid.shape
    dep = torch.empty(B, T, J, dtype=f32, device=hid.device)
    ddp = torch.empty(B, U, J, dtype=f32, device=hid.device)
    check(lib().eb_joint_hidden_bwd(_p(dhid), _p(hid), int(hid.dtype == bf16), _p(dep), _p(ddp), B, T, U, J, _s()),
          "eb_joint_hidden_bwd")
    return dep, ddp


def gemm_bf16_dtanh(A16, B16, b_mn, hid16, M, N, K):
    out = torch.empty(M, N, dtype=bf16, device=A16.device)
    with _timed("gemm_bf16_n%s" % ("n" if b_mn else "t"), 1, 2.0 * (M * K + N * K) + 4.0 * M * N, 2.0 * M * N * K):
        check(lib().eb_gemm_bf16_dtanh(_p(A16), 0, _p(B16), int(b_mn), _p(out), _p(hid16), M, N, K, _s()),
              "eb_gemm_bf16_dtanh")
    return out


def joint_dpre_reduce(dpre16):
    B, T, U, J = dpre16.shape
    dep = torch.empty(B, T, J, dtype=f32, device=dpre16.device)
    ddp = torch.empty(B, U, J, dtype=f32, device=dpre16.device)
    check(lib().eb_joint_dpre_reduce(_p(dpre16), _p(dep), _p(ddp), B, T, U, J, _s()), "eb_joint_dpre_reduce")
    PROF.launches += 1
    return dep, ddp


def rnnt_workspace(B, T, U, dtype, device):
    n = lib().eb_rnnt_workspace_bytes(B, T, U, 8 if dtype == torch.float64 else 4)
    return torch.empty(n, dtype=torch.uint8, device=device)


def rnnt_loss_fwd(logits, labels, xlen, ylen, blank, need_beta=True):
    B, T, U, V = logits.shape
    ds = 8 if logits.dtype == torch.float64 else 4
    ws = rnnt_workspace(B, T, U, logits.dtype, logits.device)
    costs = torch.empty(B, dtype=logits.dtype, device=logits.device)
    with _timed("rnnt_loss_fwd", 3, float(ds) * B * T * U * V, 0.0):
        check(lib().eb_rnnt_loss_fwd(_p(logits), _p(labels), _p(xlen), _p(ylen), B, T, U, V, blank, ds, _p(ws),
                                     _p(costs), int(need_beta), _s()), "eb_rnnt_loss_fwd")
    return costs, ws


def rnnt_loss_bwd(logits, labels, xlen, ylen, blank, ws, gscale, host_scale, out=None, out_bf16=False):
    B, T, U, V = logits.shape
    ds = 8 if logits.dtype == torch.float64 else 4
    if out is None:
        out = torch.empty(logits.shape, dtype=bf16 if out_bf16 else logits.dtype, device=logits.device)
    per_batch = int(gscale is not None and gscale.numel() > 1)
    with _timed("rnnt_loss_bwd", 1, float(ds + out.element_size()) * B * T * U * V, 0.0):
        check(lib().eb_rnnt_loss_bwd(_p(logits), _p(out), int(out.dtype == bf16), _p(labels), _p(xlen), _p(ylen), B, T,
                                     U, V, blank, ds, _p(ws), _p(gscale), per_batch, float(host_scale), _s()),
              "eb_rnnt_loss_bwd")
    return out


def joint_logits_lse(hid16, w2_16, b2, labels, xlen, ylen, B, T, U, blank):
    V, J = w2_16.shape
    logits16 = torch.empty(B, T, U, V, dtype=bf16, device=hid16.device)
    ws = rnnt_workspace(B, T, U, f32, hid16.device)
    n = B * T * U
    wsf = ws.view(f32)
    N = float(n) * V
    with _timed("joint_logits_lse", 1, 2.0 * n * J + 2.0 * N, 2.0 * N * J):
        check(lib().eb_joint_logits_lse(_p(hid16), _p(w2_16), _p(b2), _p(logits16), _p(labels), _p(xlen), _p(ylen),
                                        _p(wsf[0:n]), _p(wsf[n:2 * n]), _p(wsf[2 * n:3 * n]), B, T, U, V, J, blank,
                                        _s()), "eb_joint_logits_lse")
    return logits16, ws


def rnnt_lattice(xlen, ylen, B, T, U, ws, need_beta=True):
    costs = torch.empty(B, dtype=f32, device=ws.device)
    with _timed("rnnt_loss_fwd", 2, 0.0, 0.0):
        check(lib().eb_rnnt_loss_lattice(_p(xlen), _p(ylen), B, T, U, _p(ws), _p(costs), int(need_beta), _s()),
              "eb_rnnt_loss_lattice")
    return costs


def rnnt_loss_bwd_bf16(logits16, labels, xlen, ylen, blank, ws, gscale, host_scale):
    B, T, U, V = logits16.shape
    per_batch = int(gscale is not None and gscale.numel() > 1)
    with _timed("rnnt_loss_bwd", 1, 4.0 * B * T * U * V, 0.0):
        check(lib().eb_rnnt_loss_bwd_bf16(_p(logits16), _p(logits16), _p(labels), _p(xlen), _p(ylen), B, T, U, V, blank,
                                          _p(ws), _p(gscale), per_batch, float(host_scale), _s()), "eb_rnnt_loss_bwd_bf16")
    return logits16


def adam_step(p, g, m, v, lr, beta1, beta2, eps, weight_decay, step, grad_scale=1.0):
    check(lib().eb_adam_step(_p(p), _p(g), _p(m), _p(v), p.numel(), lr, beta1, beta2, eps, weight_decay, step,
                             grad_scale, _s()), "eb_adam_step")


def adam_step_ex(p, g, m, v, lr, beta1, beta2, eps, weight_decay, step, grad_scale=1.0, sumsq=None, max_norm=0.0,
                 adamw=False):
    check(lib().eb_adam_step_ex(_p(p), _p(g), _p(m), _p(v), p.numel(), lr, beta1, beta2, eps, weight_decay, step,
                                grad_scale, _p(sumsq), float(max_norm or 0.0), int(adamw), _s()), "eb_adam_step_ex")


def sumsq(x, out):
    check(lib().eb_sumsq(_p(x), x.numel(), _p(out), _s()), "eb_sumsq")


def logmel_frontend(x, basis, fbT, n_fft, hop, n_mels, n_stack, preemph, take_log=True, pad_to_divisible=True):
    _need(x, f32, "x")
    B, L = x.shape
    nb = n_fft // 2 + 1
    pad = n_fft // 2
    R = -(-(L + 2 * pad) // hop)
    Lp = R * hop
    F = 1 + L // hop
    seq_len = -(-L // hop)
    dev = x.device
    xp = torch.zeros(B * Lp + n_fft, dtype=f32, device=dev)
    check(lib().eb_fe_preemph_pad(_p(x), _p(xp), B, L, Lp, pad, float(preemph or 0.0), int(preemph is not None), _s()),
          "eb_fe_preemph_pad")
    rows = B * R
    spec = gemm_f32(xp, hop, 1, basis, 2 * nb, 1, rows, 2 * nb, n_fft)
    power = torch.empty(rows, nb, dtype=f32, device=dev)
    check(lib().eb_fe_power(_p(spec), _p(power), rows, nb, _s()), "eb_fe_power")
    mel = gemm_f32(power, nb, 1, fbT, n_mels, 1, rows, n_mels, nb)
    Fs = F if pad_to_divisible else F - F % n_stack
    T = -(-Fs // n_stack)
    out = torch.empty(B, T, n_mels * n_stack, dtype=f32, device=dev)
    check(lib().eb_fe_log_stack(_p(mel), _p(out), B, R, Fs, seq_len, n_mels, n_stack, T, int(take_log), _s()),
          "eb_fe_log_stack")
    return out


def fe_mask(x, spans, axis, fill=0.0):
    _need(x, f32, "x")
    B, D1, D2 = x.shape
    check(lib().eb_fe_mask(_p(x), _p(spans), B, D1, D2, spans.shape[1], axis, float(fill), _s()), "eb_fe_mask")
    return x
```

Before: 11160.

## Add ping-pong warpgroup GEMM kernel for joint LSE and dtanh epilogues

Introduces a dedicated ping-pong kernel with one producer warp and two consumer warpgroups that alternate row blocks. While one warpgroup runs its epilogue, the other runs its MMAs. The joint logits+LSE GEMM and the dhidden*dtanh GEMM now use this kernel instead of the generic persistent kernel with fused epilogues, aiming to hide the heavy exp/reduction and tanh-derivative epilogue work behind tensor-core work. It also strips debug printf from the timeout traps, which may reduce register or code pressure, and adds profiling tags. The risk is extra complexity from named barriers and register reallocation, plus possible occupancy or correctness issues in the new schedule.

Result: faster. 11510, median of 6 (+3.1%).

```diff
diff --git a/edgedict_b200/csrc/common.cuh b/edgedict_b200/csrc/common.cuh
--- a/edgedict_b200/csrc/common.cuh
+++ b/edgedict_b200/csrc/common.cuh
@@ -86,10 +86,7 @@
         if ((++spins & 0xFFFF) == 0) {
             const long long now = clock64();
             if (t0 == 0) t0 = now;
-            else if (now - t0 > 8000000000LL) {
-                printf("[edgedict_b200] grid barrier timeout: block %d saw %u, wants %u\n", blockIdx.x, v, target);
-                __trap();
-            }
+            else if (now - t0 > 8000000000LL) __trap();
         }
     }
 }
diff --git a/edgedict_b200/csrc/gemm_tc.cu b/edgedict_b200/csrc/gemm_tc.cu
--- a/edgedict_b200/csrc/gemm_tc.cu
+++ b/edgedict_b200/csrc/gemm_tc.cu
@@ -46,7 +46,99 @@
     *reinterpret_cast<__nv_bfloat162*>(p) = __floats2bfloat162_rn(a, b);
 }
 
-template <bool A_MN, bool B_MN, int BN_, bool LSE = false, bool LOW_ = false>
+struct LseRows {
+    float rm[2] = {-INFINITY, -INFINITY}, rs[2] = {0.f, 0.f}, xb[2] = {0.f, 0.f}, xl[2] = {0.f, 0.f};
+    int lab[2] = {-1, -1};
+    bool cell_ok[2] = {false, false};
+};
+
+template <int BN>
+__device__ __forceinline__ void lse_epilogue(float (&acc)[BN / 2], LseRows& s, long m0, int r_in, int n0, int nb,
+                                             int num_n, long M, int N, const float* __restrict__ bias,
+                                             __nv_bfloat16* const Ch, const LseArgs& lse, int cq, bool vec2) {
+    constexpr float LOG2E = 1.4426950408889634f;
+    if (nb == 0) {
+#pragma unroll
+        for (int h = 0; h < 2; ++h) {
+            s.rm[h] = -INFINITY; s.rs[h] = 0.f; s.xb[h] = 0.f; s.xl[h] = 0.f; s.lab[h] = -1; s.cell_ok[h] = false;
+            const long cell = m0 + r_in + 8 * h;
+            if (cell < M) {
+                const int u = (int)(cell % lse.maxU);
+                const long bt = cell / lse.maxU;
+                const int t = (int)(bt % lse.maxT), b = (int)(bt / lse.maxT);
+                const int Tn = lse.xlen[b], Un = lse.ylen[b] + 1;
+                s.cell_ok[h] = t < Tn && u < Un;
+                if (s.cell_ok[h] && u < Un - 1) s.lab[h] = lse.labels[b * (lse.maxU - 1) + u];
+            }
+        }
+    }
+#pragma unroll
+    for (int h = 0; h < 2; ++h) {
+        float cm = -INFINITY;
+#pragma unroll
+        for (int i = 0; i < BN / 8; ++i) {
+            const int col = n0 + 8 * i + cq;
+            float v0 = acc[4 * i + 2 * h], v1 = acc[4 * i + 2 * h + 1];
+            v0 = col < N ? v0 + (bias ? __ldg(bias + col) : 0.f) : -INFINITY;
+            v1 = col + 1 < N ? v1 + (bias ? __ldg(bias + col + 1) : 0.f) : -INFINITY;
+            acc[4 * i + 2 * h] = v0; acc[4 * i + 2 * h + 1] = v1;
+            cm = fmaxf(cm, fmaxf(v0, v1));
+            if (col == lse.blank) s.xb[h] = v0;
+            if (col + 1 == lse.blank) s.xb[h] = v1;
+            if (col == s.lab[h]) s.xl[h] = v0;
+            if (col + 1 == s.lab[h]) s.xl[h] = v1;
+        }
+        const float nm = fmaxf(s.rm[h], cm);
+        if (nm != -INFINITY) {
+            const float nml = nm * LOG2E;
+            float a0 = 0.f, a1 = 0.f;
+#pragma unroll
+            for (int i = 0; i < BN / 8; ++i) {
+                a0 += fast_ex2(fmaf(acc[4 * i + 2 * h], LOG2E, -nml));
+                a1 += fast_ex2(fmaf(acc[4 * i + 2 * h + 1], LOG2E, -nml));
+            }
+            s.rs[h] = s.rs[h] * fast_ex2((s.rm[h] - nm) * LOG2E) + (a0 + a1);
+            s.rm[h] = nm;
+        }
+        const long row = m0 + r_in + 8 * h;
+        if (row < M) {
+#pragma unroll
+            for (int i = 0; i < BN / 8; ++i) {
+                const int col = n0 + 8 * i + cq;
+                __nv_bfloat16* cp = Ch + row * N + col;
+                if (vec2 && col + 1 < N) st_bf16x2(cp, acc[4 * i + 2 * h], acc[4 * i + 2 * h + 1]);
+                else {
+                    if (col < N) cp[0] = __float2bfloat16(acc[4 * i + 2 * h]);
+                    if (col + 1 < N) cp[1] = __float2bfloat16(acc[4 * i + 2 * h + 1]);
+                }
+            }
+        }
+    }
+    if (nb == num_n - 1) {
+#pragma unroll
+        for (int h = 0; h < 2; ++h) {
+#pragma unroll
+            for (int o = 1; o <= 2; o <<= 1) {
+                const float m2 = __shfl_xor_sync(0xffffffffu, s.rm[h], o), s2 = __shfl_xor_sync(0xffffffffu, s.rs[h], o);
+                s.xb[h] += __shfl_xor_sync(0xffffffffu, s.xb[h], o);
+                s.xl[h] += __shfl_xor_sync(0xffffffffu, s.xl[h], o);
+                const float m = fmaxf(s.rm[h], m2);
+                s.rs[h] = (s.rm[h] == -INFINITY ? 0.f : s.rs[h] * fast_ex2((s.rm[h] - m) * LOG2E)) +
+                          (m2 == -INFINITY ? 0.f : s2 * fast_ex2((m2 - m) * LOG2E));
+                s.rm[h] = m;
+            }
+            if ((cq == 0) && s.cell_ok[h]) {
+                const long cell = m0 + r_in + 8 * h;
+                const float d = -(s.rm[h] + logf(s.rs[h]));
+                lse.denom[cell] = d;
+                lse.lpb[cell] = d + s.xb[h];
+                lse.lpl[cell] = d + s.xl[h];
+            }
+        }
+    }
+}
+
+template <bool A_MN, bool B_MN, int BN_, bool LOW_ = false>
 __global__ void __launch_bounds__(NTHREADS, LOW_ ? 2 : 1)
 gemm_tc_kernel(const __grid_constant__ CUtensorMap tma_a, const __grid_constant__ CUtensorMap tma_b,
                void* __restrict__ Cout, int c_bf16, const float* __restrict__ bias, int accumulate,
@@ -65,7 +157,7 @@
     Sched sch;
     sch.num_m = num_m; sch.num_n = num_n; sch.ksplit = ksplit; sch.out_tiles = num_m * num_n;
     sch.wid = blockIdx.x; sch.nw = gridDim.x;
-    sch.n_inner = LSE || ((ksplit == 1) && (num_m >= 2L * sch.nw));
+    sch.n_inner = (ksplit == 1) && (num_m >= 2L * sch.nw);
     const int nkb_total = (int)((K + BK - 1) / BK);
     const int kb_per = (nkb_total + ksplit - 1) / ksplit;
 
@@ -113,9 +205,6 @@
     float acc[NACC];
     int stage = 0; uint32_t phase = 0;
     long mb; int nb, ks;
-    float rm[2] = {-INFINITY, -INFINITY}, rs[2] = {0.f, 0.f}, xb[2] = {0.f, 0.f}, xl[2] = {0.f, 0.f};
-    int lab[2] = {-1, -1};
-    bool cell_ok[2] = {false, false};
     for (long jj = 0; sch.get(jj, mb, nb, ks); ++jj) {
         const int kb0 = ks * kb_per, kb1 = min(nkb_total, kb0 + kb_per);
         const long m0 = mb * BM;
@@ -144,161 +233,190 @@
         wgmma_fence_regs(acc);
         if (prev >= 0 && lane == 0) mbar_arrive(empty0 + 8 * prev);
 
-        if constexpr (LSE) {
-            constexpr float LOG2E = 1.4426950408889634f;
-            if (nb == 0) {
-#pragma unroll
-                for (int h = 0; h < 2; ++h) {
-                    rm[h] = -INFINITY; rs[h] = 0.f; xb[h] = 0.f; xl[h] = 0.f; lab[h] = -1; cell_ok[h] = false;
-                    const long cell = m0 + r_in + 8 * h;
-                    if (cell < M) {
-                        const int u = (int)(cell % lse.maxU);
-                        const long bt = cell / lse.maxU;
-                        const int t = (int)(bt % lse.maxT), b = (int)(bt / lse.maxT);
-                        const int Tn = lse.xlen[b], Un = lse.ylen[b] + 1;
-                        cell_ok[h] = t < Tn && u < Un;
-                        if (cell_ok[h] && u < Un - 1) lab[h] = lse.labels[b * (lse.maxU - 1) + u];
+        const bool add_bias = bias && ks == 0;
+        if (ksplit > 1) Cf = part + (long)ks * M * N;
+        const int acc_c = ksplit > 1 ? 0 : accumulate;
+#pragma unroll
+        for (int h = 0; h < 2; ++h) {
+            const long row = m0 + r_in + 8 * h;
+            if (row >= M) continue;
+#pragma unroll
+            for (int i = 0; i < BN / 8; ++i) {
+                const int col = n0 + 8 * i + cq;
+                if (col >= N) break;
+                const bool two = col + 1 < N, pair = two && vec2;
+                float v0 = acc[4 * i + 2 * h], v1 = acc[4 * i + 2 * h + 1];
+                if (add_bias) { v0 += __ldg(bias + col); if (two) v1 += __ldg(bias + col + 1); }
+                const long off = row * N + col;
+                if (c_bf16) {
+                    __nv_bfloat16* cp = Ch + off;
+                    if (pair) {
+                        if (accumulate) {
+                            const float2 o = __bfloat1622float2(*reinterpret_cast<const __nv_bfloat162*>(cp));
+                            v0 += o.x; v1 += o.y;
+                        }
+                        st_bf16x2(cp, v0, v1);
+                    } else {
+                        if (accumulate) { v0 += __bfloat162float(cp[0]); if (two) v1 += __bfloat162float(cp[1]); }
+                        cp[0] = __float2bfloat16(v0);
+                        if (two) cp[1] = __float2bfloat16(v1);
+                    }
+                } else {
+                    float* cp = Cf + off;
+                    if (pair) {
+                        if (acc_c) { const float2 o = *reinterpret_cast<const float2*>(cp); v0 += o.x; v1 += o.y; }
+                        *reinterpret_cast<float2*>(cp) = make_float2(v0, v1);
+                    } else {
+                        if (acc_c) { v0 += cp[0]; if (two) v1 += cp[1]; }
+                        cp[0] = v0;
+                        if (two) cp[1] = v1;
                     }
                 }
             }
-#pragma unroll
-            for (int h = 0; h < 2; ++h) {
-                float cm = -INFINITY;
-#pragma unroll
-                for (int i = 0; i < BN / 8; ++i) {
-                    const int col = n0 + 8 * i + cq;
-                    float v0 = acc[4 * i + 2 * h], v1 = acc[4 * i + 2 * h + 1];
-                    v0 = col < N ? v0 + (bias ? __ldg(bias + col) : 0.f) : -INFINITY;
-                    v1 = col + 1 < N ? v1 + (bias ? __ldg(bias + col + 1) : 0.f) : -INFINITY;
-                    acc[4 * i + 2 * h] = v0; acc[4 * i + 2 * h + 1] = v1;
-                    cm = fmaxf(cm, fmaxf(v0, v1));
-                    if (col == lse.blank) xb[h] = v0;
-                    if (col + 1 == lse.blank) xb[h] = v1;
-                    if (col == lab[h]) xl[h] = v0;
-                    if (col + 1 == lab[h]) xl[h] = v1;
+        }
+    }
+}
+
+template <int BN>
+__device__ __forceinline__ void dtanh_epilogue(const float (&acc)[BN / 2], long m0, int r_in, int n0, long M, int N,
+                                               __nv_bfloat16* __restrict__ C, const __nv_bfloat16* __restrict__ hid,
+                                               int cq) {
+#pragma unroll
+    for (int h = 0; h < 2; ++h) {
+        const long row = m0 + r_in + 8 * h;
+        if (row >= M) continue;
+        __nv_bfloat162 hx[BN / 8];
+#pragma unroll
+        for (int i = 0; i < BN / 8; ++i) {
+            const int col = n0 + 8 * i + cq;
+            hx[i] = __floats2bfloat162_rn(0.f, 0.f);
+            if (col < N) hx[i] = __ldg(reinterpret_cast<const __nv_bfloat162*>(hid + row * N + col));
+        }
+#pragma unroll
+        for (int i = 0; i < BN / 8; ++i) {
+            const int col = n0 + 8 * i + cq;
+            if (col >= N) break;
+            const float2 hh = __bfloat1622float2(hx[i]);
+            const float v0 = acc[4 * i + 2 * h] * (1.f - hh.x * hh.x), v1 = acc[4 * i + 2 * h + 1] * (1.f - hh.y * hh.y);
+            st_bf16x2(C + row * N + col, v0, v1);
+        }
+    }
+}
+
+__device__ __forceinline__ void named_bar_sync(int id, int nthreads) {
+    asm volatile("bar.sync %0, %1;" :: "r"(id), "r"(nthreads) : "memory");
+}
+__device__ __forceinline__ void named_bar_arrive(int id, int nthreads) {
+    asm volatile("bar.arrive %0, %1;" :: "r"(id), "r"(nthreads) : "memory");
+}
+
+constexpr int PP_THREADS = 3 * 128;
+template <bool B_MN, bool LSE>
+__global__ void __launch_bounds__(PP_THREADS, 1)
+gemm_tc_pingpong_kernel(const __grid_constant__ CUtensorMap tma_a, const __grid_constant__ CUtensorMap tma_b,
+                        __nv_bfloat16* __restrict__ C, const float* __restrict__ bias, long M, int N, long K,
+                        LseArgs ea) {
+    using C_ = Cfg<128>;
+    constexpr int BN = 128, STAGES = C_::STAGES, STAGE_BYTES = C_::STAGE_BYTES;
+    extern __shared__ uint8_t smem_raw[];
+    uint8_t* tiles = reinterpret_cast<uint8_t*>((reinterpret_cast<uintptr_t>(smem_raw) + 1023) & ~uintptr_t(1023));
+    uint64_t* bars = reinterpret_cast<uint64_t*>(tiles + STAGES * STAGE_BYTES);
+    const uint32_t full0 = smem_u32(bars), empty0 = smem_u32(bars + STAGES);
+
+    const int warp = threadIdx.x >> 5, lane = threadIdx.x & 31;
+    const long num_m = (M + BM - 1) / BM;
+    const int num_n = (N + BN - 1) / BN;
+    const int nkb = (int)((K + BK - 1) / BK);
+    auto row_block = [&](int w, long t) { return (long)blockIdx.x + (2 * (t / num_n) + w) * (long)gridDim.x; };
+
+    if (threadIdx.x == 0) {
+        for (int s = 0; s < STAGES; ++s) { mbar_init(full0 + 8 * s, 1); mbar_init(empty0 + 8 * s, 4); }
+        asm volatile("fence.mbarrier_init.release.cluster;" ::: "memory");
+        asm volatile("prefetch.tensormap [%0];" :: "l"(&tma_a) : "memory");
+        asm volatile("prefetch.tensormap [%0];" :: "l"(&tma_b) : "memory");
+    }
+    __syncthreads();
+
+    if (warp >= 8) {
+        asm volatile("setmaxnreg.dec.sync.aligned.u32 40;\n" ::: "memory");
+        if (warp == 8 && lane == 0) {
+            int stage = 0; uint32_t phase = 0;
+            constexpr uint32_t TX = A_BYTES + C_::B_BYTES;
+            for (long j = 0;; ++j) {
+                const int w = (int)(j & 1);
+                const long t = j >> 1, mb = row_block(w, t);
+                if (mb >= num_m) {
+                    if (w == 0) break;
+                    continue;
                 }
-                const float nm = fmaxf(rm[h], cm);
-                if (nm != -INFINITY) {
-                    const float nml = nm * LOG2E;
-                    float a0 = 0.f, a1 = 0.f;
-#pragma unroll
-                    for (int i = 0; i < BN / 8; ++i) {
-                        a0 += fast_ex2(fmaf(acc[4 * i + 2 * h], LOG2E, -nml));
-                        a1 += fast_ex2(fmaf(acc[4 * i + 2 * h + 1], LOG2E, -nml));
+                const int m0 = (int)mb * BM, n0 = (int)(t % num_n) * BN;
+                for (int kb = 0; kb < nkb; ++kb) {
+                    mbar_wait(empty0 + 8 * stage, phase ^ 1);
+                    const uint32_t sa = smem_u32(tiles + stage * STAGE_BYTES), sb = sa + A_BYTES;
+                    const uint32_t fb = full0 + 8 * stage;
+                    mbar_expect_tx(fb, TX);
+                    tma_load_2d(sa, &tma_a, kb * BK, m0, fb);
+                    if (!B_MN) tma_load_2d(sb, &tma_b, kb * BK, n0, fb);
+                    else {
+#pragma unroll
+                        for (int bx = 0; bx < BN / 64; ++bx) tma_load_2d(sb + bx * 8192, &tma_b, n0 + bx * 64, kb * BK, fb);
                     }
-                    rs[h] = rs[h] * fast_ex2((rm[h] - nm) * LOG2E) + (a0 + a1);
-                    rm[h] = nm;
+                    if (++stage == STAGES) { stage = 0; phase ^= 1; }
                 }
-                const long row = m0 + r_in + 8 * h;
-                if (row < M) {
-#pragma unroll
-                    for (int i = 0; i < BN / 8; ++i) {
-                        const int col = n0 + 8 * i + cq;
-                        __nv_bfloat16* cp = Ch + row * N + col;
-                        if (vec2 && col + 1 < N) st_bf16x2(cp, acc[4 * i + 2 * h], acc[4 * i + 2 * h + 1]);
-                        else {
-                            if (col < N) cp[0] = __float2bfloat16(acc[4 * i + 2 * h]);
-                            if (col + 1 < N) cp[1] = __float2bfloat16(acc[4 * i + 2 * h + 1]);
-                        }
-                    }
-                }
-            }
-            if (nb == num_n - 1) {
-#pragma unroll
-                for (int h = 0; h < 2; ++h) {
-#pragma unroll
-                    for (int o = 1; o <= 2; o <<= 1) {
-                        const float m2 = __shfl_xor_sync(0xffffffffu, rm[h], o), s2 = __shfl_xor_sync(0xffffffffu, rs[h], o);
-                        xb[h] += __shfl_xor_sync(0xffffffffu, xb[h], o);
-                        xl[h] += __shfl_xor_sync(0xffffffffu, xl[h], o);
-                        const float m = fmaxf(rm[h], m2);
-                        rs[h] = (rm[h] == -INFINITY ? 0.f : rs[h] * fast_ex2((rm[h] - m) * LOG2E)) +
-                                (m2 == -INFINITY ? 0.f : s2 * fast_ex2((m2 - m) * LOG2E));
-                        rm[h] = m;
-                    }
-                    if ((lane & 3) == 0 && cell_ok[h]) {
-                        const long cell = m0 + r_in + 8 * h;
-                        const float d = -(rm[h] + logf(rs[h]));
-                        lse.denom[cell] = d;
-                        lse.lpb[cell] = d + xb[h];
-                        lse.lpl[cell] = d + xl[h];
-                    }
-                }
-            }
-        } else {
-            const bool add_bias = bias && ks == 0;
-            if (ksplit > 1) Cf = part + (long)ks * M * N;
-            const int acc_c = ksplit > 1 ? 0 : accumulate;
-#pragma unroll
-            for (int h = 0; h < 2; ++h) {
-                const long row = m0 + r_in + 8 * h;
-                if (row >= M) continue;
-                constexpr bool PRE = BN == 128 && !LOW_;
-                __nv_bfloat162 hx[PRE ? BN / 8 : 1];
-                if constexpr (PRE) {
-                    if (c_bf16 && lse.aux) {
-#pragma unroll
-                        for (int i = 0; i < BN / 8; ++i) {
-                            const int col = n0 + 8 * i + cq;
-                            const long off = row * N + col;
-                            hx[i] = __floats2bfloat162_rn(0.f, 0.f);
-                            if (col + 1 < N && vec2) hx[i] = __ldg(reinterpret_cast<const __nv_bfloat162*>(lse.aux + off));
-                            else if (col < N) {
-                                hx[i].x = lse.aux[off];
-                                if (col + 1 < N) hx[i].y = lse.aux[off + 1];
-                            }
-                        }
-                    }
-                }
-#pragma unroll
-                for (int i = 0; i < BN / 8; ++i) {
-                    const int col = n0 + 8 * i + cq;
-                    if (col >= N) break;
-                    const bool two = col + 1 < N, pair = two && vec2;
-                    float v0 = acc[4 * i + 2 * h], v1 = acc[4 * i + 2 * h + 1];
-                    if (add_bias) { v0 += __ldg(bias + col); if (two) v1 += __ldg(bias + col + 1); }
-                    const long off = row * N + col;
-                    if (c_bf16) {
-                        __nv_bfloat16* cp = Ch + off;
-                        if (lse.aux) {
-                            float h0, h1 = 0.f;
-                            if constexpr (PRE) {
-                                const float2 hh = __bfloat1622float2(hx[i]);
-                                h0 = hh.x;
-                                if (two) h1 = hh.y;
-                            } else if (pair) {
-                                const float2 hh = __bfloat1622float2(__ldg(reinterpret_cast<const __nv_bfloat162*>(lse.aux + off)));
-                                h0 = hh.x; h1 = hh.y;
-                            } else {
-                                h0 = __bfloat162float(lse.aux[off]);
-                                if (two) h1 = __bfloat162float(lse.aux[off + 1]);
-                            }
-                            v0 *= 1.f - h0 * h0; v1 *= 1.f - h1 * h1;
-                        }
-                        if (pair) {
-                            if (accumulate) {
-                                const float2 o = __bfloat1622float2(*reinterpret_cast<const __nv_bfloat162*>(cp));
-                                v0 += o.x; v1 += o.y;
-                            }
-                            st_bf16x2(cp, v0, v1);
-                        } else {
-                            if (accumulate) { v0 += __bfloat162float(cp[0]); if (two) v1 += __bfloat162float(cp[1]); }
-                            cp[0] = __float2bfloat16(v0);
-                            if (two) cp[1] = __float2bfloat16(v1);
-                        }
-                    } else {
-                        float* cp = Cf + off;
-                        if (pair) {
-                            if (acc_c) { const float2 o = *reinterpret_cast<const float2*>(cp); v0 += o.x; v1 += o.y; }
-                            *reinterpret_cast<float2*>(cp) = make_float2(v0, v1);
-                        } else {
-                            if (acc_c) { v0 += cp[0]; if (two) v1 += cp[1]; }
-                            cp[0] = v0;
-                            if (two) cp[1] = v1;
-                        }
-                    }
-                }
-            }
+            }
+        }
+        return;
+    }
+
+    asm volatile("setmaxnreg.inc.sync.aligned.u32 232;\n" ::: "memory");
+    const int wg = warp >> 2;
+    const int r_in = 16 * (warp & 3) + (lane >> 2);
+    const int cq = 2 * (lane & 3);
+    const bool vec2 = (N % 2) == 0;
+    float acc[2][64];
+    LseRows rows[2];
+    int stage = 0; uint32_t phase = 0;
+    for (long t = 0;; ++t) {
+        const long mb = row_block(wg, t);
+        if (mb >= num_m) break;
+        const int nb = (int)(t % num_n);
+        const long m0 = mb * BM;
+        const int n0 = nb * BN;
+        if (wg == 1 || (t > 0 && row_block(1, t - 1) < num_m)) {
+            const int s2 = stage + nkb;
+            phase ^= (uint32_t)(s2 / STAGES) & 1u;
+            stage = s2 % STAGES;
+            named_bar_sync(1 + wg, 256);
+        }
+#pragma unroll
+        for (int i = 0; i < 64; ++i) { acc[0][i] = 0.f; acc[1][i] = 0.f; }
+        int prev = -1;
+        for (int kb = 0; kb < nkb; ++kb) {
+            mbar_wait(full0 + 8 * stage, phase);
+            const uint32_t sa = smem_u32(tiles + stage * STAGE_BYTES), sb = sa + A_BYTES;
+            wgmma_fence();
+#pragma unroll
+            for (int k = 0; k < BK / UMMA_K; ++k) {
+                const uint64_t bd = B_MN ? make_desc(sb + k * 2048, 8192, 1024) : make_desc(sb + k * 32, 16, 1024);
+                wgmma_m64n128k16<0, B_MN ? 1 : 0>(acc[0], make_desc(sa + k * 32, 16, 1024), bd, 1);
+                wgmma_m64n128k16<0, B_MN ? 1 : 0>(acc[1], make_desc(sa + 8192 + k * 32, 16, 1024), bd, 1);
+            }
+            wgmma_commit();
+            wgmma_wait<1>();
+            if (prev >= 0 && lane == 0) mbar_arrive(empty0 + 8 * prev);
+            prev = stage;
+            if (++stage == STAGES) { stage = 0; phase ^= 1; }
+        }
+        if (wg == 0 ? row_block(1, t) < num_m : row_block(0, t + 1) < num_m) named_bar_arrive(2 - wg, 256);
+        wgmma_wait<0>();
+        wgmma_fence_regs(acc[0]);
+        wgmma_fence_regs(acc[1]);
+        if (prev >= 0 && lane == 0) mbar_arrive(empty0 + 8 * prev);
+
+#pragma unroll
+        for (int hf = 0; hf < 2; ++hf) {
+            if constexpr (LSE) lse_epilogue<BN>(acc[hf], rows[hf], m0, 64 * hf + r_in, n0, nb, num_n, M, N, bias, C, ea, cq, vec2);
+            else dtanh_epilogue<BN>(acc[hf], m0, 64 * hf + r_in, n0, M, N, C, ea.aux, cq);
         }
     }
 }
@@ -325,11 +443,11 @@
     return ksplit;
 }
 
-template <bool A_MN, bool B_MN, int BN_, bool LSE, bool LOW_>
+template <bool A_MN, bool B_MN, int BN_, bool LOW_>
 int launch_kernel(const CUtensorMap& ta, const CUtensorMap& tb, void* C, int c_bf16, const float* bias, int accumulate,
                   long M, int N, long K, int ksplit, long work, const LseArgs& ea, cudaStream_t st, float* part = nullptr) {
     using C_ = Cfg<BN_, LOW_>;
-    auto kern = gemm_tc_kernel<A_MN, B_MN, BN_, LSE, LOW_>;
+    auto kern = gemm_tc_kernel<A_MN, B_MN, BN_, LOW_>;
     static bool attr_done = false;
     if (!attr_done) {
         EB_CUDA(cudaFuncSetAttribute(kern, cudaFuncAttributeMaxDynamicSharedMemorySize, C_::SMEM_BYTES));
@@ -349,12 +467,10 @@
 
 template <bool A_MN, bool B_MN, int BN_>
 int launch(const CUtensorMap& ta, const CUtensorMap& tb, void* C, int c_bf16, const float* bias, int accumulate,
-           long M, int N, long K, int ksplit, float* part, cudaStream_t st, const void* aux = nullptr) {
-    LseArgs ea = LseArgs();
-    ea.aux = reinterpret_cast<const __nv_bfloat16*>(aux);
+           long M, int N, long K, int ksplit, float* part, cudaStream_t st) {
     const long out_tiles = ((M + BM - 1) / BM) * ((N + BN_ - 1) / BN_);
-    return launch_kernel<A_MN, B_MN, BN_, false, false>(ta, tb, C, c_bf16, bias, accumulate, M, N, K, ksplit,
-                                                        out_tiles * ksplit, ea, st, part);
+    return launch_kernel<A_MN, B_MN, BN_, false>(ta, tb, C, c_bf16, bias, accumulate, M, N, K, ksplit, out_tiles * ksplit,
+                                                 LseArgs(), st, part);
 }
 
 void plan(int a_mn_major, int c_bf16, int accumulate, long M, int N, long K, int flags, bool& wide, int& ksplit) {
@@ -379,12 +495,24 @@
 int launch_low(const CUtensorMap& ta, const CUtensorMap& tb, void* C, int c_bf16, const float* bias, int accumulate,
                long M, int N, long K, cudaStream_t st) {
     const long tiles = ((M + BM - 1) / BM) * ((N + 127) / 128);
-    return launch_kernel<false, false, 128, false, true>(ta, tb, C, c_bf16, bias, accumulate, M, N, K, 1, tiles, LseArgs(), st);
-}
-
-int launch_lse(const CUtensorMap& ta, const CUtensorMap& tb, void* C, const float* bias, long M, int N, long K,
-               const LseArgs& lse, cudaStream_t st) {
-    return launch_kernel<false, false, 128, true, false>(ta, tb, C, 1, bias, 0, M, N, K, 1, (M + BM - 1) / BM, lse, st);
+    return launch_kernel<false, false, 128, true>(ta, tb, C, c_bf16, bias, accumulate, M, N, K, 1, tiles, LseArgs(), st);
+}
+
+template <bool B_MN, bool LSE>
+int launch_pingpong(const CUtensorMap& ta, const CUtensorMap& tb, void* C, const float* bias, long M, int N, long K,
+                    const LseArgs& ea, cudaStream_t st) {
+    constexpr int SMEM = Cfg<128>::SMEM_BYTES;
+    auto kern = gemm_tc_pingpong_kernel<B_MN, LSE>;
+    static bool attr_done = false;
+    if (!attr_done) {
+        EB_CUDA(cudaFuncSetAttribute(kern, cudaFuncAttributeMaxDynamicSharedMemorySize, SMEM));
+        attr_done = true;
+    }
+    const long num_m = (M + BM - 1) / BM;
+    const int grid = (int)(num_m < eb_num_sms() ? num_m : eb_num_sms());
+    kern<<<grid, PP_THREADS, SMEM, st>>>(ta, tb, reinterpret_cast<__nv_bfloat16*>(C), bias, M, N, K, ea);
+    EB_CHECK_LAUNCH();
+    return EB_OK;
 }
 
 }
@@ -408,7 +536,7 @@
     lse.labels = labels; lse.xlen = xlen; lse.ylen = ylen; lse.denom = denom; lse.lpb = lpb; lse.lpl = lpl;
     lse.maxT = maxT; lse.maxU = maxU; lse.blank = blank; lse.aux = nullptr;
     cudaStream_t st = reinterpret_cast<cudaStream_t>(stream);
-    return launch_lse(ta, tb, logits16, b2, M, V, J, lse, st);
+    return launch_pingpong<false, true>(ta, tb, logits16, b2, M, V, J, lse, st);
 }
 
 EB_API int eb_gemm_bf16(const void* A, int a_mn_major, const void* B, int b_mn_major, void* C, int c_bf16,
@@ -417,8 +545,8 @@
 }
 
 static int gemm_dispatch(const void* A, int a_mn_major, const void* B, int b_mn_major, void* C, int c_bf16,
-                         const float* bias, int accumulate, long M, int N, long K, int flags, const void* aux,
-                         float* partials, long partial_floats, void* stream);
+                         const float* bias, int accumulate, long M, int N, long K, int flags, float* partials,
+                         long partial_floats, void* stream);
 
 EB_API long eb_gemm_bf16_partials(int a_mn_major, int c_bf16, int accumulate, long M, int N, long K, int flags) {
     if (M <= 0 || N <= 0 || K <= 0) return 0;
@@ -431,19 +559,35 @@
 EB_API int eb_gemm_bf16_ex(const void* A, int a_mn_major, const void* B, int b_mn_major, void* C, int c_bf16,
                            const float* bias, int accumulate, long M, int N, long K, int flags, float* partials,
                            long partial_floats, void* stream) {
-    return gemm_dispatch(A, a_mn_major, B, b_mn_major, C, c_bf16, bias, accumulate, M, N, K, flags, nullptr, partials,
+    return gemm_dispatch(A, a_mn_major, B, b_mn_major, C, c_bf16, bias, accumulate, M, N, K, flags, partials,
                          partial_floats, stream);
 }
 
 EB_API int eb_gemm_bf16_dtanh(const void* A, int a_mn_major, const void* B, int b_mn_major, void* C16,
                               const void* hid16, long M, int N, long K, void* stream) {
-    if (!hid16 || (reinterpret_cast<uintptr_t>(hid16) & 7) || (reinterpret_cast<uintptr_t>(C16) & 7) || N % 4) return EB_ERR_INVALID;
-    return gemm_dispatch(A, a_mn_major, B, b_mn_major, C16, 1, nullptr, 0, M, N, K, 0, hid16, nullptr, 0, stream);
+    if (!A || !B || !C16 || !hid16 || a_mn_major || M <= 0 || N <= 0 || K <= 0 || N % 4 || K % 8 ||
+        (b_mn_major && N % 8))
+        return EB_ERR_INVALID;
+    if ((reinterpret_cast<uintptr_t>(A) & 15) || (reinterpret_cast<uintptr_t>(B) & 15) ||
+        (reinterpret_cast<uintptr_t>(hid16) & 7) || (reinterpret_cast<uintptr_t>(C16) & 7))
+        return EB_ERR_INVALID;
+    CUtensorMap ta, tb;
+    const bool ok = make_map(&ta, A, (uint64_t)K, (uint64_t)M, 128) &&
+                    (b_mn_major ? make_map(&tb, B, (uint64_t)N, (uint64_t)K, 64) : make_map(&tb, B, (uint64_t)K, (uint64_t)N, 128));
+    if (!ok) {
+        fprintf(stderr, "[edgedict_b200] cuTensorMapEncodeTiled failed\n");
+        return EB_ERR_CUDA;
+    }
+    LseArgs ea = LseArgs();
+    ea.aux = reinterpret_cast<const __nv_bfloat16*>(hid16);
+    cudaStream_t st = reinterpret_cast<cudaStream_t>(stream);
+    return b_mn_major ? launch_pingpong<true, false>(ta, tb, C16, nullptr, M, N, K, ea, st)
+                      : launch_pingpong<false, false>(ta, tb, C16, nullptr, M, N, K, ea, st);
 }
 
 static int gemm_dispatch(const void* A, int a_mn_major, const void* B, int b_mn_major, void* C, int c_bf16,
-                         const float* bias, int accumulate, long M, int N, long K, int flags, const void* aux,
-                         float* partials, long partial_floats, void* stream) {
+                         const float* bias, int accumulate, long M, int N, long K, int flags, float* partials,
+                         long partial_floats, void* stream) {
     if (!A || !B || !C || M <= 0 || N <= 0 || K <= 0) return EB_ERR_INVALID;
     const bool low = (flags & EB_GEMM_CORESIDENT) != 0;
     if (low && (a_mn_major || b_mn_major)) return EB_ERR_INVALID;
@@ -452,7 +596,6 @@
     bool wide;
     int ksplit;
     plan(a_mn_major, c_bf16, accumulate, M, N, K, flags, wide, ksplit);
-    if (aux) wide = false;
     if (ksplit > 1) {
         const long fit = (partials && (reinterpret_cast<uintptr_t>(partials) & 7) == 0) ? partial_floats / (M * (long)N) : 0;
         if (fit < ksplit) ksplit = fit > 1 ? (int)fit : 1;
@@ -468,8 +611,8 @@
     cudaStream_t st = reinterpret_cast<cudaStream_t>(stream);
     if (low) return launch_low(ta, tb, C, c_bf16, bias, accumulate, M, N, K, st);
 #define EB_GO(AM, BMN)                                                                                          \
-    return wide ? launch<AM, BMN, 256>(ta, tb, C, c_bf16, bias, accumulate, M, N, K, ksplit, partials, st, aux) \
-                : launch<AM, BMN, 128>(ta, tb, C, c_bf16, bias, accumulate, M, N, K, ksplit, partials, st, aux)
+    return wide ? launch<AM, BMN, 256>(ta, tb, C, c_bf16, bias, accumulate, M, N, K, ksplit, partials, st) \
+                : launch<AM, BMN, 128>(ta, tb, C, c_bf16, bias, accumulate, M, N, K, ksplit, partials, st)
     if (a_mn_major) {
         if (b_mn_major) { EB_GO(true, true); }
         EB_GO(true, false);
diff --git a/edgedict_b200/csrc/sm90.cuh b/edgedict_b200/csrc/sm90.cuh
--- a/edgedict_b200/csrc/sm90.cuh
+++ b/edgedict_b200/csrc/sm90.cuh
@@ -21,11 +21,7 @@
     do {
         asm volatile("{\n .reg .pred p;\n mbarrier.try_wait.parity.shared::cta.b64 p, [%1], %2;\n"
                      " selp.u32 %0, 1, 0, p;\n}\n" : "=r"(ok) : "r"(bar), "r"(parity) : "memory");
-        if (!ok && ++spins > (1ull << 26)) {
-            printf("[edgedict_b200] mbarrier wait timeout (block %d warp %d)\n", blockIdx.x,
-                   threadIdx.x >> 5);
-            __trap();
-        }
+        if (!ok && ++spins > (1ull << 26)) __trap();
     } while (!ok);
 }
 __device__ __forceinline__ void tma_load_2d(uint32_t dst, const CUtensorMap* map, int c0, int c1, uint32_t bar) {
@@ -136,10 +132,7 @@
     do {
         asm volatile("{\n .reg .pred p;\n mbarrier.try_wait.parity.acquire.cluster.shared::cta.b64 p, [%1], %2;\n"
                      " selp.u32 %0, 1, 0, p;\n}\n" : "=r"(ok) : "r"(bar), "r"(parity) : "memory");
-        if (!ok && ++spins > (1ull << 26)) {
-            printf("[edgedict_b200] cluster mbarrier wait timeout (block %d warp %d)\n", blockIdx.x, threadIdx.x >> 5);
-            __trap();
-        }
+        if (!ok && ++spins > (1ull << 26)) __trap();
     } while (!ok);
 }
 __device__ __forceinline__ void cluster_sync_all() {
diff --git a/edgedict_b200/functional.py b/edgedict_b200/functional.py
--- a/edgedict_b200/functional.py
+++ b/edgedict_b200/functional.py
@@ -511,9 +511,9 @@
         if db2 is None:
             db2 = ops.colsum(dlog2)
         if p == "bf16" and V % 256 == 0:
-            dw2 = ops.mm_tn(hid2, dl16, p, dy16=hid2, x16=dl16).t().contiguous()
-        else:
-            dw2 = ops.mm_tn(dlog2, hid2, p, dy16=dl16, x16=hid2 if p == "bf16" else None)
+            dw2 = ops.mm_tn(hid2, dl16, p, dy16=hid2, x16=dl16, tag="joint_dw2").t().contiguous()
+        else:
+            dw2 = ops.mm_tn(dlog2, hid2, p, dy16=dl16, x16=hid2 if p == "bf16" else None, tag="joint_dw2")
         return dw2, db2
 
     side = None
diff --git a/edgedict_b200/ops.py b/edgedict_b200/ops.py
--- a/edgedict_b200/ops.py
+++ b/edgedict_b200/ops.py
@@ -150,13 +150,13 @@
     return gemm_f32(dy, N, 1, w, w.stride(0), w.stride(1), M, K, N)
 
 
-def mm_tn(dy, x, precision="fp32", dy16=None, x16=None, out=None, accumulate=False):
+def mm_tn(dy, x, precision="fp32", dy16=None, x16=None, out=None, accumulate=False, tag=None):
     M, N = dy.shape
     K = x.shape[1]
     if precision == "bf16":
         dy16 = dy16 if dy16 is not None else (dy if dy.dtype == bf16 else cast_bf16(dy))
         x16 = x16 if x16 is not None else (x if x.dtype == bf16 else cast_bf16(x))
-        return gemm_bf16(dy16, 1, x16, 1, N, K, M, out=out, accumulate=accumulate)
+        return gemm_bf16(dy16, 1, x16, 1, N, K, M, out=out, accumulate=accumulate, tag=tag)
     _need(dy, f32, "dy")
     _need(x, f32, "x")
     return gemm_f32(dy, 1, N, x, K, 1, N, K, M, out=out, beta=1.0 if accumulate else 0.0)
@@ -523,7 +523,7 @@
 
 def gemm_bf16_dtanh(A16, B16, b_mn, hid16, M, N, K):
     out = torch.empty(M, N, dtype=bf16, device=A16.device)
-    with _timed("gemm_bf16_n%s" % ("n" if b_mn else "t"), 1, 2.0 * (M * K + N * K) + 4.0 * M * N, 2.0 * M * N * K):
+    with _timed("joint_dhidden_dtanh", 1, 2.0 * (M * K + N * K) + 4.0 * M * N, 2.0 * M * N * K):
         check(lib().eb_gemm_bf16_dtanh(_p(A16), 0, _p(B16), int(b_mn), _p(out), _p(hid16), M, N, K, _s()),
               "eb_gemm_bf16_dtanh")
     return out
```
